# AllenInstitute/distributed-vae

Measured on AMD Instinct MI355X. Metric: cells/sec per train step (fwd+loss+bwd+opt), higher is better.
Workload: dtype f32; 1 GPU; cpl_mixVAE A=2 arms, synthetic-10x-v1 50000 cells x 5000 genes per GPU, batch 5000/GPU, fp32, H=100 L=10 C=92 S=2, x_drop=0.5, Adam lr=1e-3; global_batch=5000, parallelism=dp1, noise=in-kernel Philox4x32-10

## Files before the change

distributed-vae_amd/csrc/gemm_bf16.hip:

```cpp
#include "common.hpp"

namespace mmvae {

typedef __bf16 bf16x8 __attribute__((ext_vector_type(8)));
typedef __bf16 bf16x2 __attribute__((ext_vector_type(2)));
typedef unsigned int u32x4v __attribute__((ext_vector_type(4)));


constexpr int BT = 128;
constexpr int KT = 64;
constexpr int LDB = 36;
constexpr int LDK = 136;

template <int NP>
struct Eng {
    static constexpr int KT = NP == 1 ? 64 : 32;
    static constexpr int NQ = KT / 8;
    static constexpr int LDB = KT / 2 + 4;
    static constexpr int PLANE = BT * LDB;
    static constexpr int LDK = NP == 1 ? 136 : 160;
    static constexpr int NBUF = NP == 1 ? 2 : 1;
};

__device__ __forceinline__ unsigned pack_bf16(float a, float b) {
    bf16x2 v;
    v[0] = (__bf16)a;
    v[1] = (__bf16)b;
    return __builtin_bit_cast(unsigned, v);
}

struct Operand {
    const float* ptr;
    int64_t ld;
    int rows, K;
    int kminor;
    const uint32_t* bits;
    int wpr;
    int ones_row;
    const unsigned short* pl;
    int64_t pl_plane, pl_arm;
    int pl_ld;
    const unsigned* rowmap;
    int64_t nrec;
    int map_n;
    int src16;
};

template <bool BITS, int NQ = 8>
struct TileRegsT {
    float4 v[NQ];
    uint32_t wd[BITS ? NQ : 1];
};

struct OperandDev {
    __amdgpu_buffer_rsrc_t rs, rb;
    __amdgpu_buffer_rsrc_t rm;
    const unsigned* mp;
    int ld, rows, K, wpr, ones_row;
    bool bits;
    float4 bn_sub, bn_mul;
};
template <bool KMINOR>
__device__ __forceinline__ OperandDev make_operand_dev(const Operand& o) {
    OperandDev d;
    const int64_t n = KMINOR ? (int64_t)o.K * o.ld : (int64_t)o.rows * o.ld;
    d.rs = __builtin_amdgcn_make_buffer_rsrc(const_cast<float*>(o.ptr), 0, (int)((o.rowmap ? o.nrec : n) * (o.src16 ? 2 : 4)), 0x00020000);
    d.rm = __builtin_amdgcn_make_buffer_rsrc(const_cast<unsigned*>(o.rowmap ? o.rowmap : reinterpret_cast<const unsigned*>(o.ptr)), 0,
                                             (int)((o.rowmap ? o.map_n : 1) * 4), 0x00020000);
    d.mp = o.rowmap;
    d.bits = o.bits != nullptr;
    const int64_t nb = (KMINOR ? (int64_t)o.K : (int64_t)o.rows) * o.wpr;
    d.rb = __builtin_amdgcn_make_buffer_rsrc(const_cast<uint32_t*>(d.bits ? o.bits : reinterpret_cast<const uint32_t*>(o.ptr)), 0,
                                             (int)((d.bits ? nb : 1) * 4), 0x00020000);
    d.ld = (int)o.ld; d.rows = o.rows; d.K = o.K; d.wpr = o.wpr; d.ones_row = o.ones_row;
    return d;
}

template <bool KMINOR, int NP>
__device__ __forceinline__ void piece_ph(int q, int& p, int& h) {
    if (!KMINOR && NP != 1) { p = q; h = 0; }
    else { p = q >> 1; h = q & 1; }
}
template <bool KMINOR, bool BITS = true, int NP = 1>
__device__ __forceinline__ void quad_load(TileRegsT<BITS, Eng<NP>::NQ>& t, const OperandDev& o, int r0, int k0, int kend, int q) {
    const int tid = threadIdx.x & 255;
    int p, h;
    piece_ph<KMINOR, NP>(q, p, h);
    int off, woff;
    if (!KMINOR) {
        const int row = r0 + (tid >> 3) + 32 * p;
        const int rc = min(row, o.rows - 1);
        const int k = k0 + ((tid & 7) + 8 * h) * 4;
        const bool ok = row < o.rows && k + 3 < kend && k + 3 < o.K;
        off = rc * o.ld + (ok ? k : 0);
        woff = rc * o.wpr + ((ok ? k : 0) >> 5);
    } else {
        const int k = k0 + 2 * ((tid >> 5) + 8 * p) + h;
        const int kc = min(k, o.K - 1);
        const int row = r0 + (tid & 31) * 4;
        off = kc * o.ld + (row < o.ld ? row : 0);
        woff = kc * o.wpr + (min(row, o.rows - 1) >> 5);
    }
    t.v[q] = __builtin_bit_cast(float4, __builtin_amdgcn_raw_buffer_load_b128(o.rs, off * 4, 0, 0));
    if constexpr (BITS) t.wd[q] = o.bits ? (uint32_t)__builtin_amdgcn_raw_buffer_load_b32(o.rb, woff * 4, 0, 0) : 0xFFFFFFFFu;
}

template <bool KMINOR, int NP>
__device__ __forceinline__ void quad_load_idx(TileRegsT<true, Eng<NP>::NQ>& t, const OperandDev& o, int r0, int k0, int kend, int q,
                                              const unsigned (&ro)[Eng<NP>::NQ]) {
    const int tid = threadIdx.x & 255;
    int p, h;
    piece_ph<KMINOR, NP>(q, p, h);
    int off, woff;
    if (!KMINOR) {
        const int row = r0 + (tid >> 3) + 32 * p;
        const int rc = min(row, o.rows - 1);
        const int k = k0 + ((tid & 7) + 8 * h) * 4;
        const bool ok = row < o.rows && k + 3 < kend && k + 3 < o.K;
        off = (int)ro[q] + (ok ? k : 0);
        woff = rc * o.wpr + ((ok ? k : 0) >> 5);
    } else {
        const int k = k0 + 2 * ((tid >> 5) + 8 * p) + h;
        const int kc = min(k, o.K - 1);
        const int row = r0 + (tid & 31) * 4;
        off = (int)ro[q] + (row < o.ld ? row : 0);
        woff = kc * o.wpr + (min(row, o.rows - 1) >> 5);
    }
    t.v[q] = __builtin_bit_cast(float4, __builtin_amdgcn_raw_buffer_load_b128(o.rs, off * 4, 0, 0));
    t.wd[q] = o.bits ? (uint32_t)__builtin_amdgcn_raw_buffer_load_b32(o.rb, woff * 4, 0, 0) : 0xFFFFFFFFu;
}
typedef unsigned mapw4 __attribute__((ext_vector_type(4)));
typedef const mapw4 __attribute__((address_space(4)))* map4_ptr;
template <int NP>
struct MapRegs { mapw4 s[Eng<NP>::KT / 16]; };
template <int NP>
__device__ __forceinline__ void map_request(MapRegs<NP>& mr, const OperandDev& o, int k0) {
    const int wv = __builtin_amdgcn_readfirstlane((int)(threadIdx.x & 255) >> 6);
    const unsigned* base = o.mp + __builtin_amdgcn_readfirstlane(k0) + 4 * wv;
#pragma unroll
    for (int p = 0; p < Eng<NP>::KT / 16; ++p) mr.s[p] = *(map4_ptr)(const void*)(base + 16 * p);
}
template <int NP>
__device__ __forceinline__ void map_offsets(unsigned (&ro)[Eng<NP>::NQ], const MapRegs<NP>& mr) {
    const bool hi = (threadIdx.x & 32) != 0;
#pragma unroll
    for (int q = 0; q < Eng<NP>::NQ; ++q) {
        const int p = q >> 1, h = q & 1;
        ro[q] = hi ? mr.s[p][2 + h] : mr.s[p][h];
    }
}
template <int NP>
__device__ __forceinline__ void ro_init(unsigned (&ro)[Eng<NP>::NQ], const OperandDev& o, int r0) {
    const int tid = threadIdx.x & 255;
#pragma unroll
    for (int q = 0; q < Eng<NP>::NQ; ++q) {
        int p, h;
        piece_ph<false, NP>(q, p, h);
        ro[q] = (unsigned)__builtin_amdgcn_raw_buffer_load_b32(o.rm, min(r0 + (tid >> 3) + 32 * p, o.rows - 1) * 4, 0, 0);
    }
}
template <bool KMINOR, int NP>
__device__ __forceinline__ void idx_begin(unsigned (&ro)[Eng<NP>::NQ], MapRegs<NP>& mr, const OperandDev& o, int r0, int kfirst) {
    if constexpr (KMINOR) {
        map_request<NP>(mr, o, kfirst);
        map_offsets<NP>(ro, mr);
        map_request<NP>(mr, o, kfirst + Eng<NP>::KT);
    } else ro_init<NP>(ro, o, r0);
}
template <bool KMINOR, int NP>
__device__ __forceinline__ void idx_next(unsigned (&ro)[Eng<NP>::NQ], MapRegs<NP>& mr, const OperandDev& o, int kld) {
    if constexpr (KMINOR) {
        map_offsets<NP>(ro, mr);
        map_request<NP>(mr, o, kld + Eng<NP>::KT);
    }
}
template <bool KMINOR, bool BITS = true, int NP = 1, bool BN = false>
__device__ __forceinline__ void quad_store(unsigned* __restrict__ T, const TileRegsT<BITS, Eng<NP>::NQ>& t, const OperandDev& o, int r0,
                                           int k0, int kend, int q) {
    constexpr int LDBv = Eng<NP>::LDB, PLANE = Eng<NP>::PLANE;
    const int tid = threadIdx.x & 255;
    int p, h;
    piece_ph<KMINOR, NP>(q, p, h);
    float x[4];
    int idx;
    if (!KMINOR) {
        const int kq = tid & 7, rr = tid >> 3;
        const int row = r0 + rr + 32 * p;
        const int k = k0 + (kq + 8 * h) * 4;
        const bool ok = row < o.rows && k + 3 < kend && k + 3 < o.K;
        const int nib = ok ? (BITS ? (int)(t.wd[q] >> (k & 31)) : 0xF) : 0;
        const float4 v = t.v[q];
        const float vv[4] = {v.x, v.y, v.z, v.w};
#pragma unroll
        for (int e = 0; e < 4; ++e) x[e] = __uint_as_float(__float_as_uint(vv[e]) & (unsigned)__builtin_amdgcn_sbfe(nib, e, 1));
        idx = (rr + 32 * p) * LDBv + (kq + 8 * h) * 2;
    } else {
        const int r4 = (tid & 31) * 4, kp = tid >> 5;
        const int kl = 2 * (kp + 8 * p) + h, k = k0 + kl;
        const bool kok = k < kend && k < o.K;
        const int nrow = min(max(o.rows - (r0 + r4), 0), 4);
        const int nib = kok ? ((BITS ? (int)(t.wd[q] >> ((r0 + r4) & 31)) : 0xF) & ((1 << nrow) - 1)) : 0;
        const float4 v = t.v[q];
        const float vv[4] = {v.x, v.y, v.z, v.w};
#pragma unroll
        for (int e = 0; e < 4; ++e) x[e] = __uint_as_float(__float_as_uint(vv[e]) & (unsigned)__builtin_amdgcn_sbfe(nib, e, 1));
        if constexpr (BN) {
            const float sb[4] = {o.bn_sub.x, o.bn_sub.y, o.bn_sub.z, o.bn_sub.w}, ml[4] = {o.bn_mul.x, o.bn_mul.y, o.bn_mul.z, o.bn_mul.w};
#pragma unroll
            for (int e = 0; e < 4; ++e) x[e] = ((nib >> e) & 1) ? (x[e] - sb[e]) * ml[e] : 0.f;
        }
        if (o.ones_row >= 0) {
#pragma unroll
            for (int e = 0; e < 4; ++e)
                if (kok && r0 + r4 + e == o.ones_row) x[e] = 1.f;
        }
        idx = (kl * Eng<NP>::LDK + r4) >> 1;
    }
    if constexpr (NP == 1) {
        uint2 w;
        w.x = pack_bf16(x[0], x[1]);
        w.y = pack_bf16(x[2], x[3]);
        *reinterpret_cast<uint2*>(&T[idx]) = w;
    } else {
        unsigned w0[3], w1[3];
        split3(x[0], x[1], w0);
        split3(x[2], x[3], w1);
#pragma unroll
        for (int pl = 0; pl < 3; ++pl) *reinterpret_cast<uint2*>(&T[pl * PLANE + idx]) = make_uint2(w0[pl], w1[pl]);
    }
}

struct OctRegs { u32x4v v[4]; uint32_t wd[4]; };
template <bool KMINOR, bool IDX>
__device__ __forceinline__ void oct_load(OctRegs& t, const OperandDev& o, int r0, int k0, int kend, int p, const unsigned (&ro)[8]) {
    const int tid = threadIdx.x & 255;
    int off, woff;
    if (!KMINOR) {
        const int row = r0 + (tid >> 3) + 32 * p;
        const int rc = min(row, o.rows - 1);
        const int k = k0 + 8 * (tid & 7);
        const bool ok = row < o.rows && k + 7 < kend && k + 7 < o.K;
        off = (IDX ? (int)ro[p] : rc * o.ld) + (ok ? k : 0);
        woff = rc * o.wpr + ((ok ? k : 0) >> 5);
    } else {
        const int k = k0 + (tid >> 4) + 16 * p;
        const int kc = min(k, o.K - 1);
        const int row = r0 + 8 * (tid & 15);
        off = (IDX ? (int)ro[p] : kc * o.ld) + (row < o.ld ? row : 0);
        woff = kc * o.wpr + (min(row, o.rows - 1) >> 5);
    }
    t.v[p] = __builtin_bit_cast(u32x4v, __builtin_amdgcn_raw_buffer_load_b128(o.rs, off * 2, 0, 0));
    t.wd[p] = o.bits ? (uint32_t)__builtin_amdgcn_raw_buffer_load_b32(o.rb, woff * 4, 0, 0) : 0xFFFFFFFFu;
}
template <bool KMINOR>
__device__ __forceinline__ void oct_store(unsigned* __restrict__ T, const OctRegs& t, const OperandDev& o, int r0, int k0, int kend, int p) {
    const int tid = threadIdx.x & 255;
    int byte, idx;
    if (!KMINOR) {
        const int rr = (tid >> 3) + 32 * p, row = r0 + rr;
        const int k = k0 + 8 * (tid & 7);
        const bool ok = row < o.rows && k + 7 < kend && k + 7 < o.K;
        byte = ok ? (int)((t.wd[p] >> (k & 31)) & 0xFFu) : 0;
        idx = rr * LDB + 4 * (tid & 7);
    } else {
        const int kl = (tid >> 4) + 16 * p, k = k0 + kl;
        const int r8 = 8 * (tid & 15);
        const bool kok = k < kend && k < o.K;
        const int nrow = min(max(o.rows - (r0 + r8), 0), 8);
        byte = kok ? (int)((t.wd[p] >> ((r0 + r8) & 31)) & ((1u << nrow) - 1u)) : 0;
        idx = (kl * LDK + r8) >> 1;
    }
    u32x4v w;
#pragma unroll
    for (int j = 0; j < 4; ++j) {
        const unsigned m = ((unsigned)__builtin_amdgcn_sbfe(byte, 2 * j, 1) & 0xFFFFu) | ((unsigned)__builtin_amdgcn_sbfe(byte, 2 * j + 1, 1) & 0xFFFF0000u);
        w[j] = t.v[p][j] & m;
    }
    *reinterpret_cast<u32x4v*>(&T[idx]) = w;
}
__device__ __forceinline__ void oct_ro_init(unsigned (&ro)[8], const OperandDev& o, int r0) {
    const int tid = threadIdx.x & 255;
#pragma unroll
    for (int p = 0; p < 4; ++p) ro[p] = (unsigned)__builtin_amdgcn_raw_buffer_load_b32(o.rm, min(r0 + (tid >> 3) + 32 * p, o.rows - 1) * 4, 0, 0);
}
__device__ __forceinline__ void oct_map_offsets(unsigned (&ro)[8], const MapRegs<1>& mr) {
    const int qq = (threadIdx.x >> 4) & 3;
#pragma unroll
    for (int p = 0; p < 4; ++p) {
        const unsigned lo = (qq & 1) ? mr.s[p][1] : mr.s[p][0], hi = (qq & 1) ? mr.s[p][3] : mr.s[p][2];
        ro[p] = (qq & 2) ? hi : lo;
    }
}

template <bool KMINOR, bool BITS = true, int NP = 1>
__device__ __forceinline__ void tile_load(TileRegsT<BITS, Eng<NP>::NQ>& t, const OperandDev& o, int r0, int k0, int kend) {
#pragma unroll
    for (int q = 0; q < Eng<NP>::NQ; ++q) quad_load<KMINOR, BITS, NP>(t, o, r0, k0, kend, q);
}
template <bool KMINOR, bool BITS = true, int NP = 1>
__device__ __forceinline__ void tile_store(unsigned* __restrict__ T, const TileRegsT<BITS, Eng<NP>::NQ>& t, const OperandDev& o, int r0,
                                           int k0, int kend) {
#pragma unroll
    for (int q = 0; q < Eng<NP>::NQ; ++q) quad_store<KMINOR, BITS, NP>(T, t, o, r0, k0, kend, q);
}

typedef short s16x4 __attribute__((ext_vector_type(4)));
template <bool MINOR, int LDBv = LDB, int LDKv = LDK>
__device__ __forceinline__ bf16x8 frag8(const unsigned* T, int rb, int s, int lane) {
    if (!MINOR) {
        return __builtin_bit_cast(bf16x8, *reinterpret_cast<const u32x4v*>(T + (rb + (lane & 31)) * LDBv + 4 * (lane >> 5) + 8 * s));
    } else {
        const unsigned short* Tk = reinterpret_cast<const unsigned short*>(T);
        const int grp = lane >> 4, q = (lane & 15) >> 2, p = lane & 3;
        const unsigned short* a = Tk + (16 * s + 8 * (grp >> 1) + q) * LDKv + rb + 16 * (grp & 1) + 4 * p;
        typedef s16x4 __attribute__((address_space(3))) * lds_ptr;
        const s16x4 v0 = __builtin_amdgcn_ds_read_tr16_b64_v4i16((lds_ptr)a);
        const s16x4 v1 = __builtin_amdgcn_ds_read_tr16_b64_v4i16((lds_ptr)(a + 4 * LDKv));
        typedef short s16x8 __attribute__((ext_vector_type(8)));
        s16x8 r;
        r[0] = v0[0]; r[1] = v0[1]; r[2] = v0[2]; r[3] = v0[3];
        r[4] = v1[0]; r[5] = v1[1]; r[6] = v1[2]; r[7] = v1[3];
        return __builtin_bit_cast(bf16x8, r);
    }
}

struct PlaneRegs { u32x4v v[6]; };
struct PlaneDev { __amdgpu_buffer_rsrc_t rs; int plane, ld; };
__device__ __forceinline__ PlaneDev make_plane_dev(const Operand& o, int arm) {
    PlaneDev d;
    d.rs = __builtin_amdgcn_make_buffer_rsrc(const_cast<unsigned short*>(o.pl + (int64_t)arm * o.pl_arm), 0, (int)(3 * o.pl_plane * 2), 0x00020000);
    d.plane = (int)o.pl_plane; d.ld = o.pl_ld;
    return d;
}
template <bool KMINOR>
__device__ __forceinline__ void plane_load(PlaneRegs& t, const PlaneDev& o, int r0, int k0, int j) {
    const int tid = threadIdx.x & 255, pl = j >> 1, id = tid + 256 * (j & 1);
    int off;
    if (!KMINOR) off = pl * o.plane + (r0 + (id >> 2)) * o.ld + k0 + 8 * (id & 3);
    else off = pl * o.plane + (k0 + (id >> 4)) * o.ld + r0 + 8 * (id & 15);
    t.v[j] = __builtin_bit_cast(u32x4v, __builtin_amdgcn_raw_buffer_load_b128(o.rs, off * 2, 0, 0));
}
template <bool KMINOR>
__device__ __forceinline__ void plane_store(unsigned* __restrict__ T, const PlaneRegs& t, int j) {
    const int tid = threadIdx.x & 255, pl = j >> 1, id = tid + 256 * (j & 1);
    int idx;
    if (!KMINOR) idx = pl * Eng<3>::PLANE + (id >> 2) * Eng<3>::LDB + 4 * (id & 3);
    else idx = pl * Eng<3>::PLANE + (((id >> 4) * Eng<3>::LDK + 8 * (id & 15)) >> 1);
    *reinterpret_cast<u32x4v*>(&T[idx]) = t.v[j];
}

struct SplitJob {
    const float* src; int64_t ld, src_arm;
    int R, C, Rp, Cp, ones_col;
    unsigned short* dst; int64_t dst_arm;
    const float* col_src; int64_t col_arm;
    int tr;
};
struct XbitsJob {
    NoiseDev nz; int A, B, D, wpr; uint32_t* bits; int blocks; float* zero_p; int zero_n4;
    const int64_t* rows; unsigned* map; int64_t rows_ld, n_rows;
};
struct SplitJobs { SplitJob j[24]; int first[25]; int n; XbitsJob xb; };
__global__ __launch_bounds__(256) void k_presplit(const SplitJobs js) {
    if (js.xb.zero_n4 > 0) grid_zero(js.xb.zero_p, js.xb.zero_n4);
    if (js.xb.rows && blockIdx.z == 0) {
        for (int i = blockIdx.x * 256 + threadIdx.x; i < js.xb.B + MAP_PAD; i += gridDim.x * 256) {
            const int64_t r = i < js.xb.B ? js.xb.rows[i] : 0;
            js.xb.map[i] = (unsigned)((r < 0 ? 0 : (r >= js.xb.n_rows ? js.xb.n_rows - 1 : r)) * js.xb.rows_ld);
        }
    }
    if ((int)blockIdx.x < js.xb.blocks) {
        make_xbits_range(js.xb.nz, js.xb.A, js.xb.B, js.xb.D, js.xb.wpr, js.xb.bits,
                         ((int64_t)blockIdx.z * js.xb.blocks + blockIdx.x) * 256 + threadIdx.x, (int64_t)gridDim.z * js.xb.blocks * 256);
        return;
    }
    const int bx0 = (int)blockIdx.x - js.xb.blocks;
    int ji = 0;
    while (ji + 1 < js.n && bx0 >= js.first[ji + 1]) ++ji;
    const SplitJob& J = js.j[ji];
    const int bx = bx0 - js.first[ji], nbx = js.first[ji + 1] - js.first[ji];
    const float* src = J.src + (int64_t)blockIdx.z * J.src_arm;
    const float* col = J.col_src ? J.col_src + (int64_t)blockIdx.z * J.col_arm : nullptr;
    unsigned short* dst = J.dst + (int64_t)blockIdx.z * J.dst_arm;
    const int c8n = J.Cp >> 3;
    const int64_t plane = (int64_t)J.Rp * J.Cp;
    const bool vec = (J.ld & 3) == 0 && (J.C & 3) == 0;
    const int n = J.Rp * c8n;
    for (int i = bx * 256 + threadIdx.x; i < n; i += nbx * 256) {
        const int r = i / c8n, c0 = (i - r * c8n) * 8;
        float v[8];
        if (J.tr) {
#pragma unroll
            for (int e = 0; e < 8; ++e) v[e] = (r < J.R && c0 + e < J.C) ? src[(int64_t)(c0 + e) * J.ld + r] : 0.f;
        } else if (r < J.R && vec && c0 + 8 <= J.C) {
            const float4 a = *reinterpret_cast<const float4*>(src + (int64_t)r * J.ld + c0);
            const float4 b = *reinterpret_cast<const float4*>(src + (int64_t)r * J.ld + c0 + 4);
            v[0] = a.x; v[1] = a.y; v[2] = a.z; v[3] = a.w; v[4] = b.x; v[5] = b.y; v[6] = b.z; v[7] = b.w;
        } else {
#pragma unroll
            for (int e = 0; e < 8; ++e) {
                const int c = c0 + e;
                v[e] = (r < J.R && c < J.C) ? src[(int64_t)r * J.ld + c] : ((r < J.R && c == J.ones_col) ? (col ? col[r] : 1.f) : 0.f);
            }
        }
        unsigned w[4][3];
#pragma unroll
        for (int e = 0; e < 4; ++e) split3(v[2 * e], v[2 * e + 1], w[e]);
#pragma unroll
        for (int pl = 0; pl < 3; ++pl)
            *reinterpret_cast<uint4*>(dst + pl * plane + (int64_t)r * J.Cp + c0) = make_uint4(w[0][pl], w[1][pl], w[2][pl], w[3][pl]);
    }
}

struct SlabOut {
    float* out;
    int64_t ks_stride, arm_stride;
    int ld, M, N;
};
struct Fc11Out {
    const float* bias;
    const float* x;
    float* dz;
    float* x_rec;
    float* part;
    float coef;
    int B, D;
    const unsigned* xmap;
    int64_t x_nrec;
};

struct GemmArgs {
    Operand a, b;
    int64_t a_arm, b_arm;
    int64_t a_bits_arm, b_bits_arm;
    int64_t bias_arm;
    int M, N, K;
    int KS;
    SlabOut so;
    Fc11Out fo;
    int64_t fo_arm, fo_x_arm;
    int n11;
    int A;
};

template <bool AMINOR, bool BMINOR, int NP = 1>
__device__ __forceinline__ void mfma_ktile(f32x16 (&acc)[2][2], const unsigned* As, const unsigned* Bs, int wm, int wn, int lane) {
    constexpr int LDBv = Eng<NP>::LDB, PLANE = Eng<NP>::PLANE, NS = Eng<NP>::KT / 16;
    bf16x8 a[NP == 3 ? 2 : 1][2][NP], b[NP == 3 ? 2 : 1][2][NP];
    auto frags = [&](int s, int w) __attribute__((always_inline)) {
#pragma unroll
        for (int pl = 0; pl < NP; ++pl) {
            a[w][0][pl] = frag8<AMINOR, LDBv, Eng<NP>::LDK>(As + pl * PLANE, wm * 64, s, lane);
            a[w][1][pl] = frag8<AMINOR, LDBv, Eng<NP>::LDK>(As + pl * PLANE, wm * 64 + 32, s, lane);
            b[w][0][pl] = frag8<BMINOR, LDBv, Eng<NP>::LDK>(Bs + pl * PLANE, wn * 64, s, lane);
            b[w][1][pl] = frag8<BMINOR, LDBv, Eng<NP>::LDK>(Bs + pl * PLANE, wn * 64 + 32, s, lane);
        }
    };
    if constexpr (NP == 3) {
        frags(0, 0);
        frags(1, 1);
        __builtin_amdgcn_sched_barrier(0);
    }
#pragma unroll
    for (int s = 0; s < NS; ++s) {
        const int w = NP == 3 ? s : 0;
        if constexpr (NP != 3) frags(s, 0);
#pragma unroll
        for (int i = 0; i < 2; ++i)
#pragma unroll
            for (int j = 0; j < 2; ++j) {
                if constexpr (NP == 3) {
                    acc[i][j] = __builtin_amdgcn_mfma_f32_32x32x16_bf16(a[w][i][2], b[w][j][0], acc[i][j], 0, 0, 0);
                    acc[i][j] = __builtin_amdgcn_mfma_f32_32x32x16_bf16(a[w][i][0], b[w][j][2], acc[i][j], 0, 0, 0);
                    acc[i][j] = __builtin_amdgcn_mfma_f32_32x32x16_bf16(a[w][i][1], b[w][j][1], acc[i][j], 0, 0, 0);
                    acc[i][j] = __builtin_amdgcn_mfma_f32_32x32x16_bf16(a[w][i][1], b[w][j][0], acc[i][j], 0, 0, 0);
                    acc[i][j] = __builtin_amdgcn_mfma_f32_32x32x16_bf16(a[w][i][0], b[w][j][1], acc[i][j], 0, 0, 0);
                }
                acc[i][j] = __builtin_amdgcn_mfma_f32_32x32x16_bf16(a[w][i][0], b[w][j][0], acc[i][j], 0, 0, 0);
            }
    }
}

__device__ __forceinline__ void gemm_epilogue(const GemmArgs& g, const f32x16 (&acc)[2][2], int m0, int n0, int wm, int wn, int lane, int arm) {
    const int l31 = lane & 31;
    float* out = g.so.out + (int64_t)blockIdx.y * g.so.ks_stride + (int64_t)arm * g.so.arm_stride;
#pragma unroll
    for (int i = 0; i < 2; ++i)
#pragma unroll
        for (int j = 0; j < 2; ++j) {
            const int col = n0 + 64 * wn + 32 * j + l31;
#pragma unroll
            for (int r = 0; r < 16; ++r) {
                const int row = m0 + 64 * wm + 32 * i + acc_row(r, lane);
                if (row < g.so.M && col < g.so.N) out[(int64_t)row * g.so.ld + col] = acc[i][j][r];
            }
        }
}

template <bool AMINOR, bool BMINOR, int IDX = 0, int S16 = 0>
__global__ __launch_bounds__(256, 2) void k_bf16_gemm(const GemmArgs g_in) {
    const GemmArgs g = g_in;
    __shared__ __attribute__((aligned(16))) unsigned As[2][BT * LDB];
    __shared__ __attribute__((aligned(16))) unsigned Bs[2][BT * LDB];
    const int arm = blockIdx.z, tid = threadIdx.x, lane = tid & 63, wv = tid >> 6, wm = wv >> 1, wn = wv & 1;
    Operand oa_h = g.a, ob_h = g.b;
    oa_h.ptr += (int64_t)arm * g.a_arm;
    ob_h.ptr += (int64_t)arm * g.b_arm;
    if (oa_h.bits) oa_h.bits += (int64_t)arm * g.a_bits_arm;
    if (ob_h.bits) ob_h.bits += (int64_t)arm * g.b_bits_arm;
    const OperandDev oa = make_operand_dev<AMINOR>(oa_h), ob = make_operand_dev<BMINOR>(ob_h);
    const int tiles_n = cdiv(g.N, BT);
    const int wg = blockIdx.x;
    const int m0 = (wg / tiles_n) * BT, n0 = (wg % tiles_n) * BT;
    const int nkt = cdiv(g.K, KT);
    const int kb = (int)(((int64_t)blockIdx.y * nkt) / g.KS) * KT;
    const int ke = min(g.K, (int)(((int64_t)(blockIdx.y + 1) * nkt) / g.KS) * KT);
    f32x16 acc[2][2] = {{zero16(), zero16()}, {zero16(), zero16()}};
    TileRegsT<true> ta, tb;
    OctRegs t16a, t16b;
    unsigned ro[Eng<1>::NQ] = {};
    MapRegs<1> mr = {};
    static_assert(IDX == 0 || S16 == 0 || (S16 & IDX) != 0, "row map and bf16 storage: the indexed operand (x) is a bf16 one");
    constexpr bool A16 = (S16 & 1) != 0, B16 = (S16 & 2) != 0;
    auto stage = [&](unsigned* Ad, unsigned* Bd, int kst, int kld, auto load_tag) __attribute__((always_inline)) {
        constexpr bool LOAD = decltype(load_tag)::value;
        if constexpr (LOAD && IDX == 1 && AMINOR) {
            if constexpr (A16) { oct_map_offsets(ro, mr); map_request<1>(mr, oa, kld + KT); }
            else idx_next<AMINOR, 1>(ro, mr, oa, kld);
        }
        if constexpr (LOAD && IDX == 2 && BMINOR) {
            if constexpr (B16) { oct_map_offsets(ro, mr); map_request<1>(mr, ob, kld + KT); }
            else idx_next<BMINOR, 1>(ro, mr, ob, kld);
        }
#pragma unroll
        for (int q = 0; q < 8; ++q) {
            if constexpr (A16) {
                if (q < 4) {
                    oct_store<AMINOR>(Ad, t16a, oa, m0, kst, ke, q);
                    if constexpr (LOAD) oct_load<AMINOR, IDX == 1>(t16a, oa, m0, kld, ke, q, ro);
                }
            } else {
                quad_store<AMINOR>(Ad, ta, oa, m0, kst, ke, q);
                if constexpr (LOAD) {
                    if constexpr (IDX == 1) quad_load_idx<AMINOR, 1>(ta, oa, m0, kld, ke, q, ro);
                    else quad_load<AMINOR>(ta, oa, m0, kld, ke, q);
                }
            }
            if constexpr (B16) {
                if (q < 4) {
                    oct_store<BMINOR>(Bd, t16b, ob, n0, kst, ke, q);
                    if constexpr (LOAD) oct_load<BMINOR, IDX == 2>(t16b, ob, n0, kld, ke, q, ro);
                }
            } else {
                quad_store<BMINOR>(Bd, tb, ob, n0, kst, ke, q);
                if constexpr (LOAD) {
                    if constexpr (IDX == 2) quad_load_idx<BMINOR, 1>(tb, ob, n0, kld, ke, q, ro);
                    else quad_load<BMINOR>(tb, ob, n0, kld, ke, q);
                }
            }
        }
    };
    auto first = [&](auto a_tag) __attribute__((always_inline)) {
        constexpr bool ISA = decltype(a_tag)::value;
        constexpr bool MINOR = ISA ? AMINOR : BMINOR;
        constexpr bool IDXD = IDX == (ISA ? 1 : 2), IS16 = ISA ? A16 : B16;
        const OperandDev& o = ISA ? oa : ob;
        const int r0 = ISA ? m0 : n0;
        OctRegs& t16 = ISA ? t16a : t16b;
        if constexpr (IS16) {
            if constexpr (IDXD) {
                if constexpr (MINOR) { map_request<1>(mr, o, kb); oct_map_offsets(ro, mr); map_request<1>(mr, o, kb + KT); }
                else oct_ro_init(ro, o, r0);
            }
#pragma unroll
            for (int q = 0; q < 4; ++q) oct_load<MINOR, IDXD>(t16, o, r0, kb, ke, q, ro);
        } else if constexpr (IDXD) {
            idx_begin<MINOR, 1>(ro, mr, o, r0, kb);
#pragma unroll
            for (int q = 0; q < Eng<1>::NQ; ++q) quad_load_idx<MINOR, 1>(ISA ? ta : tb, o, r0, kb, ke, q, ro);
        } else tile_load<MINOR>(ISA ? ta : tb, o, r0, kb, ke);
    };
    if (kb < ke) {
        first(VecTag{});
        first(ScalarTag{});
    }
    if (kb < ke) {
        if (kb + KT < ke) stage(As[0], Bs[0], kb, kb + KT, VecTag{});
        else stage(As[0], Bs[0], kb, kb, ScalarTag{});
    }
    __syncthreads();
    int cur = 0;
    for (int k0 = kb; k0 < ke; k0 += KT) {
        mfma_ktile<AMINOR, BMINOR>(acc, As[cur], Bs[cur], wm, wn, lane);
        if (k0 + 2 * KT < ke) stage(As[cur ^ 1], Bs[cur ^ 1], k0 + KT, k0 + 2 * KT, VecTag{});
        else if (k0 + KT < ke) stage(As[cur ^ 1], Bs[cur ^ 1], k0 + KT, k0 + KT, ScalarTag{});
        __syncthreads();
        cur ^= 1;
    }
    gemm_epilogue(g, acc, m0, n0, wm, wn, lane, arm);
}

#ifndef X3_DEPTH
#define X3_DEPTH 1
#endif
static_assert(X3_DEPTH == 1 || X3_DEPTH == 2, "one or two K tiles in flight");
template <bool AMINOR, bool BMINOR, int SHARE, int IDX = 0>
__global__ __launch_bounds__(512, 1) void k_x3_gemm(const GemmArgs g_in) {
    static_assert(SHARE == 1 || SHARE == 2, "the two tiles of a block share one operand");
    typedef Eng<3> E;
    constexpr int KTv = E::KT;
    const GemmArgs g = g_in;
    __shared__ __attribute__((aligned(16))) unsigned As[2][3 * E::PLANE];
    __shared__ __attribute__((aligned(16))) unsigned Bs[2][3 * E::PLANE];
    const int arm = blockIdx.z, grp = threadIdx.x >> 8, tid = threadIdx.x & 255, lane = tid & 63, wv = tid >> 6, wm = wv >> 1, wn = wv & 1;
    Operand oa_h = g.a, ob_h = g.b;
    oa_h.ptr += (int64_t)arm * g.a_arm;
    ob_h.ptr += (int64_t)arm * g.b_arm;
    if (oa_h.bits) oa_h.bits += (int64_t)arm * g.a_bits_arm;
    if (ob_h.bits) ob_h.bits += (int64_t)arm * g.b_bits_arm;
    const OperandDev oa = make_operand_dev<AMINOR>(oa_h), ob = make_operand_dev<BMINOR>(ob_h);
    const int tiles_m = cdiv(g.M, BT), tiles_n = cdiv(g.N, BT);
    const int bi = blockIdx.x;
    int tm, tn;
    if (SHARE == 2) { tn = bi % tiles_n; tm = 2 * (bi / tiles_n) + grp; }
    else { tm = bi % tiles_m; tn = 2 * (bi / tiles_m) + grp; }
    const bool active = tm < tiles_m && tn < tiles_n;
    const int m0 = tm * BT, n0 = tn * BT;
    const int nkt = cdiv(g.K, KTv);
    const int kb = (int)(((int64_t)blockIdx.y * nkt) / g.KS) * KTv;
    const int ke = min(g.K, (int)(((int64_t)(blockIdx.y + 1) * nkt) / g.KS) * KTv);
    const int n = ke > kb ? cdiv(ke - kb, KTv) : 0;
    f32x16 acc[2][2] = {{zero16(), zero16()}, {zero16(), zero16()}};
    constexpr int DEPTH = X3_DEPTH;
    TileRegsT<true, E::NQ> ta_[DEPTH], tb_[DEPTH];
    unsigned ro[E::NQ] = {};
    MapRegs<3> mr = {};
    PlaneRegs ps;
    constexpr bool APL = SHARE == 1, BPL = SHARE == 2;
    const PlaneDev dp = make_plane_dev(SHARE == 1 ? g.a : g.b, arm);
    const bool do_a = SHARE != 1 || grp == 0, do_b = SHARE != 2 || grp == 0;
    auto stage = [&](unsigned* Ad, unsigned* Bd, int kst, int kld, int kpl, auto load_tag, auto loadp_tag, auto slot_tag) __attribute__((always_inline)) {
        constexpr bool LOAD = decltype(load_tag)::value, LOADP = decltype(loadp_tag)::value;
        constexpr int SLOT = decltype(slot_tag)::value;
        TileRegsT<true, E::NQ>& ta = ta_[SLOT];
        TileRegsT<true, E::NQ>& tb = tb_[SLOT];
        if constexpr (LOAD && IDX == 1) idx_next<AMINOR, 3>(ro, mr, oa, kld);
        if constexpr (LOAD && IDX == 2) idx_next<BMINOR, 3>(ro, mr, ob, kld);
#pragma unroll
        for (int i = 0; i < 6; ++i) {
            if constexpr (APL) {
                if (do_a) {
                    plane_store<AMINOR>(Ad, ps, i);
                    if constexpr (LOADP) plane_load<AMINOR>(ps, dp, m0, kpl, i);
                }
            } else if (i < E::NQ) {
                if (do_a) {
                    quad_store<AMINOR, true, 3>(Ad, ta, oa, m0, kst, ke, i);
                    if constexpr (LOAD) {
                        if constexpr (IDX == 1) quad_load_idx<AMINOR, 3>(ta, oa, m0, kld, ke, i, ro);
                        else quad_load<AMINOR, true, 3>(ta, oa, m0, kld, ke, i);
                    }
                }
            }
            if constexpr (BPL) {
                if (do_b) {
                    plane_store<BMINOR>(Bd, ps, i);
                    if constexpr (LOADP) plane_load<BMINOR>(ps, dp, n0, kpl, i);
                }
            } else if (i < E::NQ) {
                if (do_b) {
                    quad_store<BMINOR, true, 3>(Bd, tb, ob, n0, kst, ke, i);
                    if constexpr (LOAD) {
                        if constexpr (IDX == 2) quad_load_idx<BMINOR, 3>(tb, ob, n0, kld, ke, i, ro);
                        else quad_load<BMINOR, true, 3>(tb, ob, n0, kld, ke, i);
                    }
                }
            }
        }
    };
    auto first = [&](auto slot_tag, int k) __attribute__((always_inline)) {
        constexpr int SLOT = decltype(slot_tag)::value;
        TileRegsT<true, E::NQ>& ta = ta_[SLOT];
        TileRegsT<true, E::NQ>& tb = tb_[SLOT];
        if constexpr (APL) {
            if (SLOT == 0 && do_a) {
#pragma unroll
                for (int i = 0; i < 6; ++i) plane_load<AMINOR>(ps, dp, m0, k, i);
            }
        } else if (do_a) {
            if constexpr (IDX == 1) {
                if constexpr (SLOT == 0) idx_begin<AMINOR, 3>(ro, mr, oa, m0, k);
                else idx_next<AMINOR, 3>(ro, mr, oa, k);
#pragma unroll
                for (int q = 0; q < E::NQ; ++q) quad_load_idx<AMINOR, 3>(ta, oa, m0, k, ke, q, ro);
            } else tile_load<AMINOR, true, 3>(ta, oa, m0, k, ke);
        }
        if constexpr (BPL) {
            if (SLOT == 0 && do_b) {
#pragma unroll
                for (int i = 0; i < 6; ++i) plane_load<BMINOR>(ps, dp, n0, k, i);
            }
        } else if (do_b) {
            if constexpr (IDX == 2) {
                if constexpr (SLOT == 0) idx_begin<BMINOR, 3>(ro, mr, ob, n0, k);
                else idx_next<BMINOR, 3>(ro, mr, ob, k);
#pragma unroll
                for (int q = 0; q < E::NQ; ++q) quad_load_idx<BMINOR, 3>(tb, ob, n0, k, ke, q, ro);
            } else tile_load<BMINOR, true, 3>(tb, ob, n0, k, ke);
        }
    };
    if (active && n > 0) {
        first(std::integral_constant<int, 0>{}, kb);
        if constexpr (DEPTH > 1) {
            if (n > 1) first(std::integral_constant<int, DEPTH - 1>{}, kb + KTv);
        }
    }
    for (int p = 0; p <= 2 * n; ++p) {
        const int q = p - grp;
        if (active && q >= 0 && q < 2 * n) {
            const int t = q >> 1, k0 = kb + t * KTv;
            unsigned* const Ad = As[SHARE == 1 ? (t & 1) : grp];
            unsigned* const Bd = Bs[SHARE == 2 ? (t & 1) : grp];
            if (q & 1) {
                mfma_ktile<AMINOR, BMINOR, 3>(acc, Ad, Bd, wm, wn, lane);
            } else {
                const bool more = t + DEPTH < n, morep = t + 1 < n;
                const int kld = k0 + DEPTH * KTv, kpl = k0 + KTv;
                auto go = [&](auto slot_tag) __attribute__((always_inline)) {
                    if (more) stage(Ad, Bd, k0, kld, kpl, VecTag{}, VecTag{}, slot_tag);
                    else if (morep) stage(Ad, Bd, k0, k0, kpl, ScalarTag{}, VecTag{}, slot_tag);
                    else stage(Ad, Bd, k0, k0, k0, ScalarTag{}, ScalarTag{}, slot_tag);
                };
                if (DEPTH == 1 || !(t & 1)) go(std::integral_constant<int, 0>{});
                else go(std::integral_constant<int, DEPTH - 1>{});
            }
        }
        __syncthreads();
    }
    if (active) gemm_epilogue(g, acc, m0, n0, wm, wn, lane, arm);
}

__global__ __launch_bounds__(256, 2) void k_bf16_fc11(const GemmArgs g_in) {
    const GemmArgs g = g_in;
    __shared__ __attribute__((aligned(16))) unsigned Ws[2][BT * LDB];
    __shared__ __attribute__((aligned(16))) unsigned Ds[2][BT * LDB];
    __shared__ float red[8];
    const int arm = blockIdx.z, tid = threadIdx.x, lane = tid & 63, wv = tid >> 6, wm = wv >> 1, wn = wv & 1;
    const int l31 = lane & 31, hh = lane >> 5;
    Operand od_h = g.a, ow_h = g.b;
    od_h.ptr += (int64_t)arm * g.a_arm;
    ow_h.ptr += (int64_t)arm * g.b_arm;
    const OperandDev od = make_operand_dev<false>(od_h), ow = make_operand_dev<false>(ow_h);
    const int c0 = blockIdx.x * BT;
    const int tiles = cdiv(g.N, BT);
    const int t0 = (int)(((int64_t)blockIdx.y * tiles) / g.KS), t1 = (int)(((int64_t)(blockIdx.y + 1) * tiles) / g.KS);
    const int K = g.K;
    const float* xa = g.fo.x + (int64_t)arm * g.fo_x_arm;
    float* dza = g.fo.dz + (int64_t)arm * g.fo_arm;
    float* xra = g.fo.x_rec ? g.fo.x_rec + (int64_t)arm * g.fo_arm : nullptr;
    const float* bias = g.fo.bias + (int64_t)arm * g.bias_arm;
    const int B = g.fo.B, D = g.fo.D;
    {
        TileRegsT<false> t0r, t1r;
        tile_load<false, false>(t0r, od, c0, 0, K);
        tile_load<false, false>(t1r, od, c0, KT, K);
        tile_store<false, false>(Ds[0], t0r, od, c0, 0, K);
        tile_store<false, false>(Ds[1], t1r, od, c0, KT, K);
    }
    TileRegsT<false> w0, w1;
    if (t0 < t1) {
        tile_load<false, false>(w0, ow, t0 * BT, 0, K);
        tile_load<false, false>(w1, ow, t0 * BT, KT, K);
    }
    float se = 0.f;
    int mism = 0;
    for (int t = t0; t < t1; ++t) {
        const int j0 = t * BT;
        tile_store<false, false>(Ws[0], w0, ow, j0, 0, K);
        tile_store<false, false>(Ws[1], w1, ow, j0, KT, K);
        __syncthreads();
        if (t + 1 < t1) {
            tile_load<false, false>(w0, ow, j0 + BT, 0, K);
            tile_load<false, false>(w1, ow, j0 + BT, KT, K);
        }
        float4 xin[2][4], b4[2][4];
        auto request = [&](int pc, float4 (&X)[4], float4 (&Bq)[4]) __attribute__((always_inline)) {
            const int i = pc >> 1, j = pc & 1;
            const int cell = c0 + 64 * wn + 32 * j + l31;
            const int64_t rowoff = (int64_t)min(cell, B - 1) * D;
#pragma unroll
            for (int q = 0; q < 4; ++q) {
                const int gene = j0 + 64 * wm + 32 * i + 8 * q + 4 * hh;
                const int gc = min(gene, D - 4);
                X[q] = *reinterpret_cast<const float4*>(xa + rowoff + gc);
                Bq[q] = *reinterpret_cast<const float4*>(bias + gc);
            }
        };
        request(0, xin[0], b4[0]);
        __builtin_amdgcn_sched_barrier(0);
        f32x16 acc[2][2] = {{zero16(), zero16()}, {zero16(), zero16()}};
        mfma_ktile<false, false>(acc, Ws[0], Ds[0], wm, wn, lane);
        if (K > KT) mfma_ktile<false, false>(acc, Ws[1], Ds[1], wm, wn, lane);
#pragma unroll
        for (int pc = 0; pc < 4; ++pc) {
            const int i = pc >> 1, j = pc & 1;
            if (pc + 1 < 4) request(pc + 1, xin[(pc + 1) & 1], b4[(pc + 1) & 1]);
            __builtin_amdgcn_sched_barrier(0);
            const int cell = c0 + 64 * wn + 32 * j + l31;
#pragma unroll
            for (int q = 0; q < 4; ++q) {
                const int gene = j0 + 64 * wm + 32 * i + 8 * q + 4 * hh;
                const bool ok = cell < B && gene < D;
                const float4 xq = xin[pc & 1][q], bq = b4[pc & 1][q];
                const float xv[4] = {xq.x, xq.y, xq.z, xq.w};
                const float bv[4] = {bq.x, bq.y, bq.z, bq.w};
                float xr[4], dz[4];
#pragma unroll
                for (int e = 0; e < 4; ++e) {
                    xr[e] = fmaxf(acc[i][j][4 * q + e] + bv[e], 0.f);
                    const float er = xr[e] - xv[e];
                    dz[e] = xr[e] > 0.f ? g.fo.coef * er : 0.f;
                    se += ok ? er * er : 0.f;
                    mism += (ok && ((xr[e] > 0.1f) != (xv[e] > 0.1f))) ? 1 : 0;
                }
                if (ok) {
                    *reinterpret_cast<float4*>(dza + (int64_t)cell * D + gene) = make_float4(dz[0], dz[1], dz[2], dz[3]);
                    if (xra) *reinterpret_cast<float4*>(xra + (int64_t)cell * D + gene) = make_float4(xr[0], xr[1], xr[2], xr[3]);
                }
            }
            asm volatile("" : "+v"(mism), "+v"(se));
            __builtin_amdgcn_sched_barrier(0);
        }
        __syncthreads();
    }
    se = wave_sum(se);
    const float mf = wave_sum((float)mism);
    if (lane == 0) { red[wv * 2] = se; red[wv * 2 + 1] = mf; }
    __syncthreads();
    if (tid == 0) {
        float* p = g.fo.part + ((int64_t)arm * g.n11 + (int64_t)blockIdx.x * g.KS + blockIdx.y) * 2;
        p[0] = red[0] + red[2] + red[4] + red[6];
        p[1] = red[1] + red[3] + red[5] + red[7];
    }
}

static_assert(KT == 64, "W16: a row of W11's planes (128 bf16) is exactly the two K tiles in LDS");
template <bool S16, bool W16 = false>
__global__ __launch_bounds__(256, 2) void k_bf16_fc11g(const GemmArgs g_in) {
    const GemmArgs g = g_in;
    __shared__ __attribute__((aligned(16))) unsigned Ws[2][BT * LDB];
    __shared__ __attribute__((aligned(16))) unsigned Ds[2][BT * LDB];
    __shared__ __attribute__((aligned(16))) float bias_s[BT];
    __shared__ float red[8];
    const int arm = blockIdx.z, tid = threadIdx.x, lane = tid & 63, wv = tid >> 6;
    const int l31 = lane & 31, hh = lane >> 5;
    Operand od_h = g.a, ow_h = g.b;
    od_h.ptr += (int64_t)arm * g.a_arm;
    ow_h.ptr += (int64_t)arm * g.b_arm;
    const OperandDev od = make_operand_dev<false>(od_h), ow = make_operand_dev<false>(ow_h);
    const int c0 = blockIdx.x * BT;
    const int tiles = cdiv(g.N, BT);
    const int t0 = (int)(((int64_t)blockIdx.y * tiles) / g.KS), t1 = (int)(((int64_t)(blockIdx.y + 1) * tiles) / g.KS);
    const int K = g.K;
    const int ksteps1 = K > KT ? cdiv(K - KT, 16) : 0;
    const float* xa = g.fo.x + (int64_t)arm * g.fo_x_arm;
    float* dza = g.fo.dz + (int64_t)arm * g.fo_arm;
    const float* bias = g.fo.bias + (int64_t)arm * g.bias_arm;
    const int B = g.fo.B, D = g.fo.D;
    {
        TileRegsT<false> t0r, t1r;
        tile_load<false, false>(t0r, od, c0, 0, K);
        tile_load<false, false>(t1r, od, c0, KT, K);
        tile_store<false, false>(Ds[0], t0r, od, c0, 0, K);
        tile_store<false, false>(Ds[1], t1r, od, c0, KT, K);
    }
    TileRegsT<false> w0, w1;
    OctRegs wo0, wo1;
    const unsigned no_map[8] = {0, 0, 0, 0, 0, 0, 0, 0};
    auto w_request = [&](int j) __attribute__((always_inline)) {
        if constexpr (W16) {
#pragma unroll
            for (int p = 0; p < 4; ++p) {
                oct_load<false, false>(wo0, ow, j, 0, 2 * KT, p, no_map);
                oct_load<false, false>(wo1, ow, j, KT, 2 * KT, p, no_map);
            }
        } else {
            tile_load<false, false>(w0, ow, j, 0, K);
            tile_load<false, false>(w1, ow, j, KT, K);
        }
    };
    auto w_store = [&](int j) __attribute__((always_inline)) {
        if constexpr (W16) {
#pragma unroll
            for (int p = 0; p < 4; ++p) {
                oct_store<false>(Ws[0], wo0, ow, j, 0, 2 * KT, p);
                oct_store<false>(Ws[1], wo1, ow, j, KT, 2 * KT, p);
            }
        } else {
            tile_store<false, false>(Ws[0], w0, ow, j, 0, K);
            tile_store<false, false>(Ws[1], w1, ow, j, KT, K);
        }
    };
    float bnext = 0.f;
    if (t0 < t1) {
        w_request(t0 * BT);
        if (tid < BT) bnext = bias[min(t0 * BT + tid, D - 1)];
    }
    f32x16 gd[4] = {zero16(), zero16(), zero16(), zero16()};
    float se = 0.f;
    int mism = 0;
    const int cell = c0 + 32 * wv + l31;
    const int64_t rowoff = g.fo.xmap ? (int64_t)g.fo.xmap[min(cell, B - 1)] : (int64_t)min(cell, B - 1) * D;
    const unsigned short* Wk16[2] = {reinterpret_cast<const unsigned short*>(Ws[0]), reinterpret_cast<const unsigned short*>(Ws[1])};
    typedef short s16x4 __attribute__((ext_vector_type(4)));
    typedef s16x4 __attribute__((address_space(3))) * lds_ptr;
    const int tr_off = ((lane & 15) >> 2) * (2 * LDB) + 16 * ((lane >> 4) & 1) + 4 * (lane & 3);
    for (int t = t0; t < t1; ++t) {
        const int j0 = t * BT;
        w_store(j0);
        if (tid < BT) bias_s[tid] = bnext;
        __syncthreads();
        if (t + 1 < t1) {
            w_request(j0 + BT);
            if (tid < BT) bnext = bias[min(j0 + BT + tid, D - 1)];
        }
#pragma unroll
        for (int half = 0; half < 2; ++half) {
            float4 xin[2][4];
            u32x4v xraw[2][2];
#pragma unroll
            for (int gl = 0; gl < 2; ++gl) {
                if constexpr (S16) {
#pragma unroll
                    for (int qp = 0; qp < 2; ++qp) {
                        const int gene = j0 + 32 * (2 * half + gl) + 8 * (2 * qp + hh);
                        xraw[gl][qp] = *reinterpret_cast<const u32x4v*>(reinterpret_cast<const unsigned short*>(xa) + rowoff + min(gene, D - 8));
                    }
                } else {
#pragma unroll
                    for (int q = 0; q < 4; ++q) {
                        const int gene = j0 + 32 * (2 * half + gl) + 8 * q + 4 * hh;
                        xin[gl][q] = *reinterpret_cast<const float4*>(xa + rowoff + min(gene, D - 4));
                    }
                }
            }
            __builtin_amdgcn_sched_barrier(0);
            f32x16 acc[2] = {zero16(), zero16()};
#pragma unroll
            for (int s = 0; s < KT / 16; ++s) {
                const bf16x8 b = frag8<false>(Ds[0], 32 * wv, s, lane);
                acc[0] = __builtin_amdgcn_mfma_f32_32x32x16_bf16(frag8<false>(Ws[0], 32 * (2 * half), s, lane), b, acc[0], 0, 0, 0);
                acc[1] = __builtin_amdgcn_mfma_f32_32x32x16_bf16(frag8<false>(Ws[0], 32 * (2 * half + 1), s, lane), b, acc[1], 0, 0, 0);
            }
            for (int s = 0; s < ksteps1; ++s) {
                const bf16x8 b = frag8<false>(Ds[1], 32 * wv, s, lane);
                acc[0] = __builtin_amdgcn_mfma_f32_32x32x16_bf16(frag8<false>(Ws[1], 32 * (2 * half), s, lane), b, acc[0], 0, 0, 0);
                acc[1] = __builtin_amdgcn_mfma_f32_32x32x16_bf16(frag8<false>(Ws[1], 32 * (2 * half + 1), s, lane), b, acc[1], 0, 0, 0);
            }
#pragma unroll
            for (int gl = 0; gl < 2; ++gl) {
                const int gi = 2 * half + gl;
                float dzr[16];
                if constexpr (S16) {
#pragma unroll
                    for (int qp = 0; qp < 2; ++qp) {
                        const auto s0 = __builtin_amdgcn_permlane32_swap(xraw[gl][qp][0], xraw[gl][qp][2], false, false);
                        const auto s1 = __builtin_amdgcn_permlane32_swap(xraw[gl][qp][1], xraw[gl][qp][3], false, false);
                        xin[gl][2 * qp] = make_float4(__uint_as_float(s0[0] << 16), __uint_as_float(s0[0] & 0xFFFF0000u),
                                                      __uint_as_float(s1[0] << 16), __uint_as_float(s1[0] & 0xFFFF0000u));
                        xin[gl][2 * qp + 1] = make_float4(__uint_as_float(s0[1] << 16), __uint_as_float(s0[1] & 0xFFFF0000u),
                                                          __uint_as_float(s1[1] << 16), __uint_as_float(s1[1] & 0xFFFF0000u));
                    }
                }
#pragma unroll
                for (int q = 0; q < 4; ++q) {
                    const int gene = j0 + 32 * gi + 8 * q + 4 * hh;
                    const bool ok = cell < B && gene < D;
                    const float4 xq = xin[gl][q];
                    const float4 bq = *reinterpret_cast<const float4*>(&bias_s[32 * gi + 8 * q + 4 * hh]);
                    const float xv[4] = {xq.x, xq.y, xq.z, xq.w};
                    const float bv[4] = {bq.x, bq.y, bq.z, bq.w};
#pragma unroll
                    for (int e = 0; e < 4; ++e) {
                        const float xr = fmaxf(acc[gl][4 * q + e] + bv[e], 0.f);
                        const float er = xr - xv[e];
                        dzr[4 * q + e] = (ok && xr > 0.f) ? g.fo.coef * er : 0.f;
                        se += ok ? er * er : 0.f;
                        mism += (ok && ((xr > 0.1f) != (xv[e] > 0.1f))) ? 1 : 0;
                    }
                    if constexpr (!S16) {
                        if (ok) *reinterpret_cast<float4*>(dza + (int64_t)cell * D + gene) =
                            make_float4(dzr[4 * q], dzr[4 * q + 1], dzr[4 * q + 2], dzr[4 * q + 3]);
                    }
                }
                if constexpr (S16) {
#pragma unroll
                    for (int qp = 0; qp < 2; ++qp) {
                        const int qe = 2 * qp, qo = 2 * qp + 1;
                        const auto s0 = __builtin_amdgcn_permlane32_swap(pack_bf16(dzr[4 * qe], dzr[4 * qe + 1]), pack_bf16(dzr[4 * qo], dzr[4 * qo + 1]), false, false);
                        const auto s1 = __builtin_amdgcn_permlane32_swap(pack_bf16(dzr[4 * qe + 2], dzr[4 * qe + 3]), pack_bf16(dzr[4 * qo + 2], dzr[4 * qo + 3]), false, false);
                        u32x4v w;
                        w[0] = s0[0]; w[1] = s1[0]; w[2] = s0[1]; w[3] = s1[1];
                        const int gene = j0 + 32 * gi + 8 * (2 * qp + hh);
                        if (cell < B && gene < D) *reinterpret_cast<u32x4v*>(reinterpret_cast<unsigned short*>(dza) + (int64_t)cell * D + gene) = w;
                    }
                }
#pragma unroll
                for (int c = 0; c < 2; ++c) {
                    u32x4v au;
                    au[0] = pack_bf16(dzr[8 * c + 0], dzr[8 * c + 1]);
                    au[1] = pack_bf16(dzr[8 * c + 2], dzr[8 * c + 3]);
                    au[2] = pack_bf16(dzr[8 * c + 4], dzr[8 * c + 5]);
                    au[3] = pack_bf16(dzr[8 * c + 6], dzr[8 * c + 7]);
                    const bf16x8 afr = __builtin_bit_cast(bf16x8, au);
                    const int grow = 32 * gi + 16 * c + 4 * hh;
#pragma unroll
                    for (int nt = 0; nt < 4; ++nt) {
                        const unsigned short* a = Wk16[nt >> 1] + grow * (2 * LDB) + 32 * (nt & 1) + tr_off;
                        const s16x4 v0 = __builtin_amdgcn_ds_read_tr16_b64_v4i16((lds_ptr)a);
                        const s16x4 v1 = __builtin_amdgcn_ds_read_tr16_b64_v4i16((lds_ptr)(a + 8 * (2 * LDB)));
                        typedef short s16x8 __attribute__((ext_vector_type(8)));
                        s16x8 r;
                        r[0] = v0[0]; r[1] = v0[1]; r[2] = v0[2]; r[3] = v0[3];
                        r[4] = v1[0]; r[5] = v1[1]; r[6] = v1[2]; r[7] = v1[3];
                        gd[nt] = __builtin_amdgcn_mfma_f32_32x32x16_bf16(afr, __builtin_bit_cast(bf16x8, r), gd[nt], 0, 0, 0);
                    }
                }
                asm volatile("" : "+v"(mism), "+v"(se));
                __builtin_amdgcn_sched_barrier(0);
            }
        }
        __syncthreads();
    }
    {
        const int H = g.K;
        float* out = g.so.out + (int64_t)blockIdx.y * g.so.ks_stride + (int64_t)arm * g.so.arm_stride;
#pragma unroll
        for (int nt = 0; nt < 4; ++nt) {
            const int h = 32 * nt + l31;
#pragma unroll
            for (int r = 0; r < 16; ++r) {
                const int row = c0 + 32 * wv + acc_row(r, lane);
                if (row < B && h < H) out[(int64_t)row * H + h] = gd[nt][r];
            }
        }
    }
    se = wave_sum(se);
    const float mf = wave_sum((float)mism);
    if (lane == 0) { red[wv * 2] = se; red[wv * 2 + 1] = mf; }
    __syncthreads();
    if (tid == 0) {
        float* p = g.fo.part + ((int64_t)arm * g.n11 + (int64_t)blockIdx.x * g.KS + blockIdx.y) * 2;
        p[0] = red[0] + red[2] + red[4] + red[6];
        p[1] = red[1] + red[3] + red[5] + red[7];
    }
}

constexpr int FW_ROW = 64;
constexpr int FW_PLANE = 64 * FW_ROW;
constexpr int FW_TILE = 3 * FW_PLANE;
__device__ __forceinline__ int fw_swz(int row) { return ((row & 3) << 2) | ((row >> 2) & 3); }
__global__ __launch_bounds__(256, 1) void k_x3_fc11g(const GemmArgs g_in) {
    const GemmArgs g = g_in;
    __shared__ __attribute__((aligned(16))) unsigned Wl[3 * FW_TILE];
    __shared__ float red[8];
    const int arm = blockIdx.z, tid = threadIdx.x, lane = tid & 63, wv = tid >> 6;
    const int l31 = lane & 31, hh = lane >> 5;
    const unsigned short* Wp = g.b.pl + (int64_t)arm * g.b.pl_arm;
    const unsigned short* Dp = g.a.pl + (int64_t)arm * g.a.pl_arm;
    const int64_t wplane = g.b.pl_plane, dplane = g.a.pl_plane;
    const int B = g.fo.B, D = g.fo.D, H = g.K;
    const int c0 = blockIdx.x * 128;
    const int tiles = cdiv(D, 64);
    const int t0 = (int)(((int64_t)blockIdx.y * tiles) / g.KS), t1 = (int)(((int64_t)(blockIdx.y + 1) * tiles) / g.KS);
    const int cell = c0 + 32 * wv + l31;
    const float* xa = g.fo.x + (int64_t)arm * g.fo_x_arm;
    float* dza = g.fo.dz + (int64_t)arm * g.fo_arm;
    const __amdgpu_buffer_rsrc_t rx = __builtin_amdgcn_make_buffer_rsrc(const_cast<float*>(xa), 0, (int)((g.fo.xmap ? g.fo.x_nrec : (int64_t)B * D) * 4), 0x00020000);
    const __amdgpu_buffer_rsrc_t rz = __builtin_amdgcn_make_buffer_rsrc(dza, 0, (int)((int64_t)B * D * 4), 0x00020000);
    const int rowoff = g.fo.xmap ? (int)g.fo.xmap[min(cell, B - 1)] : min(cell, B - 1) * D;
    const bool cell_ok = cell < B;
    int dzoff = min(cell, B - 1) * D * 4;
    asm volatile("" : "+v"(dzoff));
    int dlim = cell_ok ? D : 0;
    asm volatile("" : "+v"(dlim));

    const int wv_s = __builtin_amdgcn_readfirstlane(wv);
    const unsigned wl_base = (unsigned)(size_t)(__attribute__((address_space(3))) void*)(&Wl[0]);
    const int lrow = 4 * wv + (lane >> 4);
    const unsigned dma_voff = 2u * ((unsigned)lrow * 128u + 8u * (unsigned)((lane & 15) ^ fw_swz(lrow)));
    auto dma = [&](int t) __attribute__((always_inline)) {
        const int buf = (t - t0) % 3;
        const unsigned lds0 = wl_base + 4u * (unsigned)(buf * FW_TILE) + 1024u * (unsigned)wv_s;
        const unsigned short* src0 = Wp + (int64_t)t * (64 * 128);
#pragma unroll
        for (int j = 0; j < 12; ++j) {
            const unsigned short* src = src0 + (int64_t)(j >> 2) * wplane + (j & 3) * (16 * 128);
            const unsigned lds_addr = lds0 + 4u * (unsigned)((j >> 2) * FW_PLANE) + 4096u * (unsigned)(j & 3);
            asm volatile("s_mov_b32 m0, %0\n\ts_nop 0\n\tglobal_load_lds_dwordx4 %1, %2"
                         :: "s"(lds_addr), "v"(dma_voff), "s"(src) : "memory");
        }
    };
    if (t0 < t1) dma(t0);
    if (t0 + 1 < t1) dma(t0 + 1);
    bf16x8 dfr[7][3];
    {
        const int cr = min(cell, (int)(dplane / 128) - 1);
#pragma unroll
        for (int s = 0; s < 7; ++s)
#pragma unroll
            for (int pl = 0; pl < 3; ++pl)
                dfr[s][pl] = __builtin_bit_cast(bf16x8, *reinterpret_cast<const u32x4v*>(Dp + (int64_t)pl * dplane + (int64_t)cr * 128 + 16 * s + 8 * hh));
    }
    f32x16 gd[4] = {zero16(), zero16(), zero16(), zero16()};
    float seq[4] = {0.f, 0.f, 0.f, 0.f};
    int mism = 0;
    typedef s16x4 __attribute__((address_space(3))) * lds_ptr;
    typedef short s16x8 __attribute__((ext_vector_type(8)));
    const int tr_q = (lane & 15) >> 2, tr_blk = 2 * ((lane >> 4) & 1) + ((lane & 3) >> 1), tr_half = 4 * (lane & 1);
    const int npieces = 2 * (t1 - t0);
    auto w_rows = [&](int p) __attribute__((always_inline)) { return Wl + ((p >> 1) % 3) * FW_TILE + 32 * (p & 1) * FW_ROW; };
    const int a_swz = fw_swz(l31);
    auto a_frag = [&](const unsigned* Wr, int s, int pl) __attribute__((always_inline)) {
        return __builtin_bit_cast(bf16x8, *reinterpret_cast<const u32x4v*>(Wr + pl * FW_PLANE + l31 * FW_ROW + 4 * ((2 * s + hh) ^ a_swz)));
    };
    auto request_x = [&](float4 (&X)[4], int j0g, int q) __attribute__((always_inline)) {
        const int gene = j0g + 8 * q + 4 * hh;
        int off = gene < dlim ? (rowoff + gene) * 4 : -16;
        asm("" : "+v"(off));
        X[q] = __builtin_bit_cast(float4, __builtin_amdgcn_raw_buffer_load_b128(rx, off, 0, 0));
    };
    auto mfma6 = [&](f32x16& acc, const bf16x8 (&a)[3], int s) __attribute__((always_inline)) {
        acc = __builtin_amdgcn_mfma_f32_32x32x16_bf16(a[2], dfr[s][0], acc, 0, 0, 0);
        acc = __builtin_amdgcn_mfma_f32_32x32x16_bf16(a[0], dfr[s][2], acc, 0, 0, 0);
        acc = __builtin_amdgcn_mfma_f32_32x32x16_bf16(a[1], dfr[s][1], acc, 0, 0, 0);
        acc = __builtin_amdgcn_mfma_f32_32x32x16_bf16(a[1], dfr[s][0], acc, 0, 0, 0);
        acc = __builtin_amdgcn_mfma_f32_32x32x16_bf16(a[0], dfr[s][1], acc, 0, 0, 0);
        acc = __builtin_amdgcn_mfma_f32_32x32x16_bf16(a[0], dfr[s][0], acc, 0, 0, 0);
    };
    bf16x8 an[3][3];
    bf16x8 wq[2][2][3];
    auto z_frags = [&](const unsigned* Wr, int s) __attribute__((always_inline)) {
#pragma unroll
        for (int pl = 0; pl < 3; ++pl) an[s % 3][pl] = a_frag(Wr, s, pl);
    };
    auto d_frags = [&](const unsigned short* Wt16, int r) __attribute__((always_inline)) {
        const int row0 = 16 * (r >> 1) + 4 * hh + tr_q;
        const int sw0 = fw_swz(row0), sw1 = fw_swz(row0 + 8);
#pragma unroll
        for (int j = 0; j < 2; ++j)
#pragma unroll
            for (int pl = 0; pl < 3; ++pl) {
                const int blk = 4 * (2 * (r & 1) + j) + tr_blk;
                const unsigned short* base = Wt16 + pl * (2 * FW_PLANE) + tr_half;
                const s16x4 v0 = __builtin_amdgcn_ds_read_tr16_b64_v4i16((lds_ptr)(base + row0 * (2 * FW_ROW) + 8 * (blk ^ sw0)));
                const s16x4 v1 = __builtin_amdgcn_ds_read_tr16_b64_v4i16((lds_ptr)(base + (row0 + 8) * (2 * FW_ROW) + 8 * (blk ^ sw1)));
                s16x8 rr;
                rr[0] = v0[0]; rr[1] = v0[1]; rr[2] = v0[2]; rr[3] = v0[3];
                rr[4] = v1[0]; rr[5] = v1[1]; rr[6] = v1[2]; rr[7] = v1[3];
                wq[r & 1][j][pl] = __builtin_bit_cast(bf16x8, rr);
            }
    };
    float4 xa_[4], xb_[4];
    f32x16 acc_a = zero16();
    __builtin_amdgcn_s_waitcnt(0x0F70);
#pragma unroll
    for (int s7 = 0; s7 < 7; ++s7)
#pragma unroll
        for (int pl = 0; pl < 3; ++pl) asm volatile("" : "+a"(dfr[s7][pl]));
    if (npieces > 0) {
#pragma unroll
        for (int q = 0; q < 4; ++q) request_x(xa_, t0 * 64, q);
        __builtin_amdgcn_s_waitcnt(0x0F70);
#pragma unroll
        for (int q = 0; q < 4; ++q) asm volatile("" : "+v"(xa_[q].x), "+v"(xa_[q].y), "+v"(xa_[q].z), "+v"(xa_[q].w));
        __syncthreads();
        if (t0 + 2 < t1) dma(t0 + 2);
        const unsigned* Wr = w_rows(0);
#pragma unroll
        for (int s = 0; s < 7; ++s) {
            bf16x8 a[3];
#pragma unroll
            for (int pl = 0; pl < 3; ++pl) a[pl] = a_frag(Wr, s, pl);
            mfma6(acc_a, a, s);
        }
        const unsigned* W1 = w_rows(npieces > 1 ? 1 : 0);
        z_frags(W1, 0);
        z_frags(W1, 1);
    }
    auto piece = [&](int p, f32x16& accn, float4 (&xin)[4], float4 (&xnx)[4], int dma_tile) __attribute__((always_inline)) {
        const int j0g = t0 * 64 + 32 * p;
        const unsigned* Wn = w_rows(p + 1 < npieces ? p + 1 : p);
        const unsigned short* Wt16 = reinterpret_cast<const unsigned short*>(w_rows(p));
        f32x16 acc = accn;
        asm volatile("" : "+v"(acc));
        accn = zero16();
        unsigned au[2][3][4];
        float dzq[4];
#pragma unroll
        for (int q = 0; q < 4; ++q) request_x(xnx, j0g + 32, q);
        auto chunk = [&](int ch) __attribute__((always_inline)) {
            const int q = ch >> 1;
            if ((ch & 1) == 0) {
                const int gene = j0g + 8 * q + 4 * hh;
                const float xv[4] = {xin[q].x, xin[q].y, xin[q].z, xin[q].w};
#pragma unroll
                for (int e = 0; e < 4; ++e) {
                    const float a_ = acc[4 * q + e];
                    const float xr = __int_as_float(max(__float_as_int(a_), 0));
                    const float er = xr - xv[e];
                    seq[q] = __builtin_fmaf(er, er, seq[q]);
                    const float d_ = g.fo.coef * er;
                    dzq[e] = a_ > 0.f ? d_ : 0.f;
                    mism += __builtin_popcountll(__builtin_amdgcn_ballot_w64(xr > 0.1f) ^ __builtin_amdgcn_ballot_w64(xv[e] > 0.1f));
                }
                int soff = gene < dlim ? dzoff + gene * 4 : -16;
                asm("" : "+v"(soff));
                __builtin_amdgcn_raw_buffer_store_b128(__builtin_bit_cast(u32x4v, make_float4(dzq[0], dzq[1], dzq[2], dzq[3])), rz, soff, 0, 0);
            } else {
                unsigned w0[3], w1[3];
                split3(dzq[0], dzq[1], w0);
                split3(dzq[2], dzq[3], w1);
#pragma unroll
                for (int pl = 0; pl < 3; ++pl) { au[q >> 1][pl][2 * (q & 1)] = w0[pl]; au[q >> 1][pl][2 * (q & 1) + 1] = w1[pl]; }
            }
        };
#pragma unroll
        for (int q = 0; q < 4; ++q) asm volatile("" : "+v"(xin[q].x), "+v"(xin[q].y), "+v"(xin[q].z), "+v"(xin[q].w));
#pragma unroll
        for (int s = 0; s < 7; ++s) {
            __builtin_amdgcn_sched_barrier(0);
            if (s + 2 < 7) z_frags(Wn, s + 2);
            if (s == 5) d_frags(Wt16, 0);
            mfma6(accn, an[s % 3], s);
            if (s < 5) chunk(s);
        }
        asm volatile("" : "+s"(mism));
        if (dma_tile >= 0) dma(dma_tile);
#pragma unroll
        for (int r = 0; r < 4; ++r) {
            __builtin_amdgcn_sched_barrier(0);
            if (r + 1 < 4) d_frags(Wt16, r + 1);
            if (r >= 2) {
                const unsigned* W2 = w_rows(p + 2 < npieces ? p + 2 : p);
                z_frags(W2, r - 2);
            }
            if (r == 0) { chunk(5); chunk(6); }
            if (r == 1) chunk(7);
            const int c = r >> 1;
            bf16x8 af[3];
#pragma unroll
            for (int pl = 0; pl < 3; ++pl) {
                u32x4v u;
                u[0] = au[c][pl][0]; u[1] = au[c][pl][1]; u[2] = au[c][pl][2]; u[3] = au[c][pl][3];
                af[pl] = __builtin_bit_cast(bf16x8, u);
            }
            const int n0 = 2 * (r & 1);
#pragma unroll
            for (int j = 0; j < 2; ++j) gd[n0 + j] = __builtin_amdgcn_mfma_f32_32x32x16_bf16(af[2], wq[r & 1][j][0], gd[n0 + j], 0, 0, 0);
#pragma unroll
            for (int j = 0; j < 2; ++j) gd[n0 + j] = __builtin_amdgcn_mfma_f32_32x32x16_bf16(af[0], wq[r & 1][j][2], gd[n0 + j], 0, 0, 0);
#pragma unroll
            for (int j = 0; j < 2; ++j) gd[n0 + j] = __builtin_amdgcn_mfma_f32_32x32x16_bf16(af[1], wq[r & 1][j][1], gd[n0 + j], 0, 0, 0);
#pragma unroll
            for (int j = 0; j < 2; ++j) gd[n0 + j] = __builtin_amdgcn_mfma_f32_32x32x16_bf16(af[1], wq[r & 1][j][0], gd[n0 + j], 0, 0, 0);
#pragma unroll
            for (int j = 0; j < 2; ++j) gd[n0 + j] = __builtin_amdgcn_mfma_f32_32x32x16_bf16(af[0], wq[r & 1][j][1], gd[n0 + j], 0, 0, 0);
#pragma unroll
            for (int j = 0; j < 2; ++j) gd[n0 + j] = __builtin_amdgcn_mfma_f32_32x32x16_bf16(af[0], wq[r & 1][j][0], gd[n0 + j], 0, 0, 0);
        }
        __builtin_amdgcn_sched_barrier(0);
    };
    for (int t = t0; t < t1; ++t) {
        const int p = 2 * (t - t0);
        piece(p, acc_a, xa_, xb_, (t > t0 && t + 2 < t1) ? t + 2 : -1);
        piece(p + 1, acc_a, xb_, xa_, -1);
        __builtin_amdgcn_s_waitcnt(0x0F74);
        __syncthreads();
    }
    {
        float* out = g.so.out + (int64_t)blockIdx.y * g.so.ks_stride + (int64_t)arm * g.so.arm_stride;
#pragma unroll
        for (int nt = 0; nt < 4; ++nt) {
            const int h = 32 * nt + l31;
#pragma unroll
            for (int r = 0; r < 16; ++r) {
                const int row = c0 + 32 * wv + acc_row(r, lane);
                if (row < B && h < H) out[(int64_t)row * H + h] = gd[nt][r];
            }
        }
    }
    const float se = wave_sum((seq[0] + seq[1]) + (seq[2] + seq[3]));
    if (lane == 0) { red[wv * 2] = se; red[wv * 2 + 1] = (float)mism; }
    __syncthreads();
    if (tid == 0) {
        float* pp = g.fo.part + ((int64_t)arm * g.n11 + (int64_t)blockIdx.x * g.KS + blockIdx.y) * 2;
        pp[0] = (red[0] + red[2]) + (red[4] + red[6]);
        pp[1] = (red[1] + red[3]) + (red[5] + red[7]);
    }
    if (blockIdx.x == 0 && blockIdx.y == 0)
        for (int i = (int)gridDim.x * g.KS * 2 + tid; i < 2 * g.n11; i += 256) g.fo.part[(int64_t)arm * g.n11 * 2 + i] = 0.f;
}

struct Fc11OutArgs {
    const unsigned short* wpl; int64_t w_plane, w_arm;
    const unsigned short* dpl; int64_t d_plane, d_arm;
    float* out;
    int B, D, KS;
};
template <int NP, int NK>
__global__ __launch_bounds__(256, 1) void k_fc11_out(const Fc11OutArgs g) {
    const int arm = blockIdx.z, tid = threadIdx.x, lane = tid & 63, wv = tid >> 6;
    const int l31 = lane & 31, hh = lane >> 5;
    const int B = g.B, D = g.D;
    const int cell = blockIdx.x * 128 + 32 * wv + l31;
    const unsigned short* Wp = g.wpl + (int64_t)arm * g.w_arm;
    const unsigned short* Dp = g.dpl + (int64_t)arm * g.d_arm;
    bf16x8 dfr[NK][NP];
    {
        const int cr = min(cell, (int)(g.d_plane / 128) - 1);
#pragma unroll
        for (int s = 0; s < NK; ++s)
#pragma unroll
            for (int pl = 0; pl < NP; ++pl)
                dfr[s][pl] = __builtin_bit_cast(bf16x8, *reinterpret_cast<const u32x4v*>(Dp + (int64_t)pl * g.d_plane + (int64_t)cr * 128 + 16 * s + 8 * hh));
    }
    const int npc = cdiv(D, 32);
    const int p0 = (int)(((int64_t)blockIdx.y * npc) / g.KS), p1 = (int)(((int64_t)(blockIdx.y + 1) * npc) / g.KS);
    auto load_w = [&](int p, bf16x8 (&a)[NK][NP]) __attribute__((always_inline)) {
        const unsigned short* r = Wp + (int64_t)(32 * p + l31) * 128 + 8 * hh;
#pragma unroll
        for (int s = 0; s < NK; ++s)
#pragma unroll
            for (int pl = 0; pl < NP; ++pl)
                a[s][pl] = __builtin_bit_cast(bf16x8, *reinterpret_cast<const u32x4v*>(r + (int64_t)pl * g.w_plane + 16 * s));
    };
    float* orow = g.out + ((int64_t)arm * B + min(cell, B - 1)) * D;
    const bool cell_ok = cell < B;
    bf16x8 wa[NK][NP], wb[NK][NP];
    auto piece = [&](int p, const bf16x8 (&a)[NK][NP]) __attribute__((always_inline)) {
        f32x16 acc = zero16();
#pragma unroll
        for (int s = 0; s < NK; ++s) {
            if constexpr (NP == 3) {
                acc = __builtin_amdgcn_mfma_f32_32x32x16_bf16(a[s][2], dfr[s][0], acc, 0, 0, 0);
                acc = __builtin_amdgcn_mfma_f32_32x32x16_bf16(a[s][0], dfr[s][2], acc, 0, 0, 0);
                acc = __builtin_amdgcn_mfma_f32_32x32x16_bf16(a[s][1], dfr[s][1], acc, 0, 0, 0);
                acc = __builtin_amdgcn_mfma_f32_32x32x16_bf16(a[s][1], dfr[s][0], acc, 0, 0, 0);
                acc = __builtin_amdgcn_mfma_f32_32x32x16_bf16(a[s][0], dfr[s][1], acc, 0, 0, 0);
            }
            acc = __builtin_amdgcn_mfma_f32_32x32x16_bf16(a[s][0], dfr[s][0], acc, 0, 0, 0);
        }
#pragma unroll
        for (int q = 0; q < 4; ++q) {
            const int gene = 32 * p + 8 * q + 4 * hh;
            if (cell_ok && gene < D)
                *reinterpret_cast<float4*>(orow + gene) = make_float4(relu_keep_nan(acc[4 * q]), relu_keep_nan(acc[4 * q + 1]),
                                                                      relu_keep_nan(acc[4 * q + 2]), relu_keep_nan(acc[4 * q + 3]));
        }
    };
    if (p0 < p1) load_w(p0, wa);
    for (int p = p0; p < p1; p += 2) {
        if (p + 1 < p1) load_w(p + 1, wb);
        piece(p, wa);
        if (p + 1 >= p1) break;
        if (p + 2 < p1) load_w(p + 2, wa);
        piece(p + 1, wb);
    }
}

__global__ __launch_bounds__(512, 1) void k_x3_small(const TnDescs descs, int ndesc, int A, int B, int KS) {
    typedef Eng<3> E;
    constexpr int KTv = E::KT;
    __shared__ __attribute__((aligned(16))) unsigned As[2][3 * E::PLANE];
    __shared__ __attribute__((aligned(16))) unsigned Bs[2][3 * E::PLANE];
    const int grp = threadIdx.x >> 8, tid = threadIdx.x & 255, lane = tid & 63, wv = tid >> 6, wm = wv >> 1, wn = wv & 1;
    const int unit = 2 * blockIdx.x + grp;
    const bool active = unit < ndesc * A;
    const int di = active ? unit % ndesc : 0, arm = active ? unit / ndesc : 0;
    const TnDesc& dr = descs.d[di];
    const TnDesc d = {dr.P, dr.p_arm_stride, dr.ldp, dr.Mv, dr.Q, dr.q_arm_stride, dr.ldq, dr.Nv, dr.q_ones, dr.q_xmask,
                      dr.q_mean, dr.q_rstd, dr.out, dr.out_arm_stride, dr.out_ks_stride, dr.ldo};
    Operand oa_h{d.P + (int64_t)arm * d.p_arm_stride, d.ldp, d.Mv, B, 1, nullptr, 0, -1, nullptr, 0, 0, 0};
    Operand ob_h{d.Q + (int64_t)arm * d.q_arm_stride, d.ldq, d.Nv, B, 1, nullptr, 0, d.q_ones ? d.Nv : -1, nullptr, 0, 0, 0};
    OperandDev oa = make_operand_dev<true>(oa_h), ob = make_operand_dev<true>(ob_h);
    const bool bn = d.q_mean != nullptr;
    {
        const int r4 = (tid & 31) * 4;
        float sb[4] = {0.f, 0.f, 0.f, 0.f}, ml[4] = {1.f, 1.f, 1.f, 1.f};
        if (bn) {
#pragma unroll
            for (int e = 0; e < 4; ++e)
                if (r4 + e < d.Nv) { sb[e] = d.q_mean[(int64_t)arm * d.Nv + r4 + e]; ml[e] = d.q_rstd[(int64_t)arm * d.Nv + r4 + e]; }
        }
        ob.bn_sub = make_float4(sb[0], sb[1], sb[2], sb[3]);
        ob.bn_mul = make_float4(ml[0], ml[1], ml[2], ml[3]);
    }
    const int nkt = cdiv(B, KTv);
    const int kb = (int)(((int64_t)blockIdx.y * nkt) / KS) * KTv;
    const int ke = min(B, (int)(((int64_t)(blockIdx.y + 1) * nkt) / KS) * KTv);
    const int n = ke > kb ? cdiv(ke - kb, KTv) : 0;
    f32x16 acc[2][2] = {{zero16(), zero16()}, {zero16(), zero16()}};
    TileRegsT<false, E::NQ> ta, tb;
    unsigned* const Ad = As[grp];
    unsigned* const Bd = Bs[grp];
    auto stage = [&](int kst, int kld, auto load_tag) __attribute__((always_inline)) {
        constexpr bool LOAD = decltype(load_tag)::value;
#pragma unroll
        for (int i = 0; i < E::NQ; ++i) {
            quad_store<true, false, 3>(Ad, ta, oa, 0, kst, ke, i);
            if constexpr (LOAD) quad_load<true, false, 3>(ta, oa, 0, kld, ke, i);
            quad_store<true, false, 3, true>(Bd, tb, ob, 0, kst, ke, i);
            if constexpr (LOAD) quad_load<true, false, 3>(tb, ob, 0, kld, ke, i);
        }
    };
    if (active && n > 0) {
        tile_load<true, false, 3>(ta, oa, 0, kb, ke);
        tile_load<true, false, 3>(tb, ob, 0, kb, ke);
    }
    for (int p = 0; p <= 2 * n; ++p) {
        const int q = p - grp;
        if (active && q >= 0 && q < 2 * n) {
            const int k0 = kb + (q >> 1) * KTv;
            if (q & 1) mfma_ktile<true, true, 3>(acc, Ad, Bd, wm, wn, lane);
            else if (k0 + KTv < ke) stage(k0, k0 + KTv, VecTag{});
            else stage(k0, k0, ScalarTag{});
        }
        __syncthreads();
    }
    if (!active) return;
    float* out = d.out + (int64_t)blockIdx.y * d.out_ks_stride + (int64_t)arm * d.out_arm_stride;
    const int ncols = d.Nv + d.q_ones, l31 = lane & 31;
#pragma unroll
    for (int i = 0; i < 2; ++i)
#pragma unroll
        for (int j = 0; j < 2; ++j) {
            const int col = 64 * wn + 32 * j + l31;
#pragma unroll
            for (int r = 0; r < 16; ++r) {
                const int row = 64 * wm + 32 * i + acc_row(r, lane);
                if (row < d.Mv && col < ncols) out[(int64_t)row * d.ldo + col] = acc[i][j][r];
            }
        }
}

static Operand kmajor(const float* p, int64_t ld, int rows, int K) {
    Operand o{};
    o.ptr = p; o.ld = ld; o.rows = rows; o.K = K; o.ones_row = -1;
    return o;
}
static Operand kminor(const float* p, int64_t ld, int rows, int K) { Operand o = kmajor(p, ld, rows, K); o.kminor = 1; return o; }

enum { PL_W1 = 0, PL_W11 = 1, PL_D10 = 2, PL_DZ1 = 3 };
struct PlaneGeom { int R, C, Rp, Cp, ones_col; int64_t ws_off; };
static PlaneGeom plane_geom(const Ctx& c, int kind) {
    const mmvae_dims& d = c.d;
    switch (kind) {
        case PL_W1:  return PlaneGeom{d.H, d.D, 128, rup(d.D, 32), -1, c.lay.pl_w1};
        case PL_W11: return PlaneGeom{d.D, d.H, rup(d.D, 128), 128, d.H, c.lay.pl_w11};
        case PL_D10: return PlaneGeom{d.B, d.H, rup(d.B, 256), 128, d.H, c.lay.pl_d10};
        default:     return PlaneGeom{d.B, d.H, rup(d.B, 256), 128, -1, c.lay.pl_dz1};
    }
}
static void use_planes(const Ctx& c, Operand& o, int kind) {
    const PlaneGeom g = plane_geom(c, kind);
    o.pl = reinterpret_cast<const unsigned short*>(c.ws + g.ws_off);
    o.pl_plane = (int64_t)g.Rp * g.Cp; o.pl_arm = 3 * o.pl_plane; o.pl_ld = g.Cp;
}
static int64_t read_slice0_bf16(const Ctx& c, Operand& o, int kind, bool whole = false) {
    const PlaneGeom g = plane_geom(c, kind);
    o.ptr = reinterpret_cast<const float*>(c.ws + g.ws_off); o.ld = g.Cp; o.src16 = 1;
    if (whole) { o.rows = g.Rp; o.K = g.Cp; }
    return 3 * (int64_t)g.Rp * g.Cp / 2;
}
static SplitJob plane_job(const Ctx& c, int kind, const float* src, int64_t ld, int64_t src_arm, const float* col_src = nullptr, int64_t col_arm = 0) {
    const PlaneGeom g = plane_geom(c, kind);
    return SplitJob{src, ld, src_arm, g.R, g.C, g.Rp, g.Cp, g.ones_col, reinterpret_cast<unsigned short*>(c.ws + g.ws_off),
                    3 * (int64_t)g.Rp * g.Cp, col_src, col_arm};
}
static int launch_presplit(hipStream_t s, int A, const SplitJob* jobs, int n, const XbitsJob* xb = nullptr) {
    SplitJobs js{};
    if (xb) js.xb = *xb;
    js.n = n;
    for (int i = 0; i < n; ++i) {
        js.j[i] = jobs[i];
        js.first[i + 1] = js.first[i] + (int)imin64(1024, cdiv64((int64_t)jobs[i].Rp * (jobs[i].Cp / 8), 256));
    }
    hipLaunchKernelGGL(k_presplit, dim3(js.xb.blocks + js.first[n], 1, A), dim3(256), 0, s, js);
    HIP_LAUNCH_CHECK("k_presplit");
    return 0;
}

static SplitJob small_plane_job(const Ctx& c, const float* params, int s, bool transposed) {
    const int H = c.d.H, L = c.d.L, CS = c.d.C + c.d.S;
    const int ti[PL_SMALL_LAYERS] = {2, 4, 6, 8, 16, 18, 20, 22, 24};
    const int nn[PL_SMALL_LAYERS] = {H, H, H, L, L, H, H, H, H}, kk[PL_SMALL_LAYERS] = {H, H, H, H, CS, L, H, H, H};
    unsigned short* base = reinterpret_cast<unsigned short*>(c.ws + c.lay.pl_small);
    return SplitJob{params + c.po.o[ti[s]], kk[s], c.po.per_arm, transposed ? kk[s] : nn[s], transposed ? nn[s] : kk[s], 128, 128, -1,
                    base + (int64_t)(transposed ? PL_SMALL_LAYERS + s : s) * 3 * 128 * 128, (int64_t)PL_SMALL_SLOTS * 3 * 128 * 128,
                    nullptr, 0, transposed ? 1 : 0};
}

int launch_x3_planes(const Ctx& c, const float* params, bool head, const mmvae_noise* nz) {
    const Plan& p = c.plan;
    const mmvae_dims& d = c.d;
    XbitsJob xb{};
    const bool xbits = head && p.zero == ZERO_PRESPLIT;
    if (xbits) {
        xb.nz = make_noise_dev(nz, c.h);
        xb.A = d.A; xb.B = d.B; xb.D = d.D; xb.wpr = cdiv(d.D, 32);
        xb.bits = reinterpret_cast<uint32_t*>(c.ws + c.lay.xbits);
        xb.blocks = (int)imin64(2048, cdiv64((int64_t)d.B * cdiv(xb.wpr, xbits_words_per_thread(xb.nz)), 256));
        xb.zero_p = c.ws + c.lay.fc11_part;
        xb.zero_n4 = (int)(c.fwd_zero_floats() / 4);
        if (p.rowmap) {
            xb.rows = c.x_rows; xb.map = reinterpret_cast<unsigned*>(c.ws + c.lay.rowmap);
            xb.rows_ld = c.x_ld; xb.n_rows = c.x_nrows;
        }
    }
    SplitJob jobs[24];
    int n = 0;
    if (head && (p.big == GEMM_X3 || p.narrow)) {
        jobs[n++] = plane_job(c, PL_W1, params + c.po.o[0], d.D, c.po.per_arm);
        jobs[n++] = plane_job(c, PL_W11, params + c.po.o[26], d.H, c.po.per_arm, params + c.po.o[27], c.po.per_arm);
    }
    if (p.chain_planes)
        for (int s = 0; s < PL_SMALL_LAYERS; ++s) {
            jobs[n++] = small_plane_job(c, params, s, false);
            jobs[n++] = small_plane_job(c, params, s, true);
        }
    return launch_presplit(c.stream, d.A, jobs, n, xbits ? &xb : nullptr);
}

int launch_dec_planes(const Ctx& c, const float* params) {
    const Plan& p = c.plan;
    const mmvae_dims& d = c.d;
    SplitJob jobs[6];
    int n = 0;
    if (p.fc11 == FC11_OUT_X3 || p.fc11 == FC11_OUT_BF16)
        jobs[n++] = plane_job(c, PL_W11, params + c.po.o[26], d.H, c.po.per_arm, params + c.po.o[27], c.po.per_arm);
    if (p.chain_planes)
        for (int s = PL_SMALL_DEC0; s < PL_SMALL_LAYERS; ++s) jobs[n++] = small_plane_job(c, params, s, false);
    return n ? launch_presplit(c.stream, d.A, jobs, n) : 0;
}

int launch_fc11_out_bf16(const Ctx& c, float* x_rec) {
    const mmvae_dims& d = c.d;
    Operand w{}, dp{};
    use_planes(c, w, PL_W11); use_planes(c, dp, PL_D10);
    Fc11OutArgs a{};
    a.wpl = w.pl; a.w_plane = w.pl_plane; a.w_arm = w.pl_arm;
    a.dpl = dp.pl; a.d_plane = dp.pl_plane; a.d_arm = dp.pl_arm;
    a.out = x_rec;
    a.B = d.B; a.D = d.D;
    const bool x3 = c.plan.fc11 == FC11_OUT_X3;
    const int blocks = cdiv(d.B, 128) * d.A, slots = (x3 ? 1 : 2) * 256, cap = min(64, cdiv(d.D, 32));
    int ks = 1;
    double best = 0.0;
    for (int k = 1; k <= cap; ++k) {
        const int nwg = blocks * k;
        const double eff = (double)nwg / (double)(cdiv(nwg, slots) * slots);
        if (nwg >= slots && eff >= 0.9) { ks = k; break; }
        if (eff > best + 1e-9) { best = eff; ks = k; }
    }
    a.KS = ks;
    const dim3 grid(cdiv(d.B, 128), ks, d.A);
    if (x3) hipLaunchKernelGGL((k_fc11_out<3, 7>), grid, dim3(256), 0, c.stream, a);
    else hipLaunchKernelGGL((k_fc11_out<1, 8>), grid, dim3(256), 0, c.stream, a);
    HIP_LAUNCH_CHECK("k_fc11_out");
    return 0;
}

static Operand x_operand(const Ctx& c, const float* x, int64_t xs, bool minor, int64_t* arm, int64_t* bits_arm) {
    const mmvae_dims& d = c.d;
    Operand o = minor ? kminor(x, d.D, d.D, d.B) : kmajor(x, d.D, d.B, d.D);
    if (c.dropout()) { o.bits = reinterpret_cast<const uint32_t*>(c.ws + c.lay.xbits); o.wpr = cdiv(d.D, 32); }
    if (c.plan.rowmap) { o.rowmap = reinterpret_cast<const unsigned*>(c.ws + c.lay.rowmap); o.nrec = c.x_nrows * c.x_ld; o.map_n = d.B; }
    if (c.plan.rowmap && c.plan.big != GEMM_X3 && c.x16) { o.ptr = reinterpret_cast<const float*>(c.x16); o.src16 = 1; }
    *arm = xs; *bits_arm = (int64_t)d.B * o.wpr;
    return o;
}

typedef void (*GemmKernel)(const GemmArgs);
struct SlabVariant { bool x3, aminor, bminor; int share, idx, s16; GemmKernel kernel; };
#define BF16_GEMM(AMINOR, BMINOR, IDX, S16) SlabVariant{false, AMINOR, BMINOR, 0, IDX, S16, k_bf16_gemm<AMINOR, BMINOR, IDX, S16>}
#define X3_GEMM(AMINOR, BMINOR, SHARE, IDX) SlabVariant{true, AMINOR, BMINOR, SHARE, IDX, 0, k_x3_gemm<AMINOR, BMINOR, SHARE, IDX>}
static const SlabVariant slab_variants[] = {
    BF16_GEMM(false, false, 0, 0), BF16_GEMM(false, false, 1, 0), BF16_GEMM(false, false, 1, 1), BF16_GEMM(false, false, 1, 3),
    X3_GEMM(false, false, 2, 0), X3_GEMM(false, false, 2, 1),
    BF16_GEMM(false, true, 0, 0),
    BF16_GEMM(true, true, 0, 0), BF16_GEMM(true, true, 2, 0), BF16_GEMM(true, true, 2, 2), BF16_GEMM(true, true, 2, 3),
    X3_GEMM(true, true, 1, 0), X3_GEMM(true, true, 1, 2),
    BF16_GEMM(true, true, 0, 1), X3_GEMM(true, true, 2, 0),
};
#undef BF16_GEMM
#undef X3_GEMM
static int launch_slab_gemm(const Ctx& c, const GemmArgs& g, int share, dim3 grid, const char* what) {
    const bool x3 = c.plan.big == GEMM_X3, aminor = g.a.kminor != 0, bminor = g.b.kminor != 0;
    const int idx = (g.a.rowmap ? 1 : 0) | (g.b.rowmap ? 2 : 0), s16 = (g.a.src16 ? 1 : 0) | (g.b.src16 ? 2 : 0);
    if (!x3) share = 0;
    for (const SlabVariant& v : slab_variants)
        if (v.x3 == x3 && v.aminor == aminor && v.bminor == bminor && v.share == share && v.idx == idx && v.s16 == s16) {
            hipLaunchKernelGGL(v.kernel, grid, dim3(x3 ? 512 : 256), 0, c.stream, g);
            HIP_LAUNCH_CHECK(what);
            return 0;
        }
    set_error("%s: no %s kernel for A k-%s, B k-%s, share %d, row map %d, bf16 source %d", what, x3 ? "k_x3_gemm" : "k_bf16_gemm",
              aminor ? "minor" : "major", bminor ? "minor" : "major", share, idx, s16);
    return MMVAE_E_LAUNCH;
}
static dim3 slab_grid(const Ctx& c, const GemmArgs& g, int paired) {
    return dim3(c.plan.big == GEMM_X3 ? cdiv(cdiv(paired, BT), 2) : cdiv(g.M, BT) * cdiv(g.N, BT), g.KS, g.A);
}

int launch_fc1_fwd_bf16(const Ctx& c, const float* params, const float* x, int64_t xs) {
    const mmvae_dims& d = c.d;
    GemmArgs g{};
    g.a = x_operand(c, x, xs, false, &g.a_arm, &g.a_bits_arm);
    g.b = kmajor(params + c.po.o[0], d.D, d.H, d.D); g.b_arm = c.po.per_arm;
    if (c.plan.big == GEMM_X3) use_planes(c, g.b, PL_W1);
    else if (g.a.src16 && c.plan.narrow) g.b_arm = read_slice0_bf16(c, g.b, PL_W1);
    g.M = d.B; g.N = d.H; g.K = d.D; g.KS = c.lay.sp.ks_fc1; g.A = d.A;
    g.so = SlabOut{c.ws + c.lay.fc1_slab, (int64_t)d.A * d.B * NP, (int64_t)d.B * NP, NP, d.B, d.H};
    return launch_slab_gemm(c, g, 2, slab_grid(c, g, d.B), "k_bf16_gemm<fc1>");
}

static GemmArgs fc11_args(const Ctx& c, const float* params, const float* x, int64_t xs, float* x_rec) {
    const mmvae_dims& d = c.d;
    const Layout& L = c.lay;
    GemmArgs g{};
    g.a = kmajor(c.ws + L.Dk[4], d.H, d.B, d.H);
    g.b = kmajor(params + c.po.o[26], d.H, d.D, d.H);
    g.M = d.B; g.N = d.D; g.K = d.H; g.KS = L.sp.ks_gd10; g.A = d.A; g.n11 = L.n11;
    g.fo = Fc11Out{params + c.po.o[27], x, c.ws + L.DZ11, x_rec, c.ws + L.fc11_part, c.fc11_coef(), d.B, d.D, nullptr, 0};
    if (c.plan.rowmap) {
        g.fo.xmap = reinterpret_cast<const unsigned*>(c.ws + L.rowmap);
        g.fo.x_nrec = c.x_nrows * c.x_ld;
    }
    g.fo_arm = (int64_t)d.B * d.D;
    g.fo_x_arm = xs;
    return g;
}
static SlabOut gd10_slab(const Ctx& c) {
    const mmvae_dims& d = c.d;
    return SlabOut{c.ws + c.lay.GD10_slab, (int64_t)d.A * d.B * d.H, (int64_t)d.B * d.H, d.H, d.B, d.H};
}

int launch_fc11_x3(const Ctx& c, const float* params, const float* x, int64_t xs) {
    const mmvae_dims& d = c.d;
    GemmArgs g = fc11_args(c, params, x, xs, nullptr);
    use_planes(c, g.b, PL_W11);
    use_planes(c, g.a, PL_D10);
    g.so = gd10_slab(c);
    launch_k(c, c.plan.fc11_fork_rides ? c.ev(EV_FORK) : nullptr, k_x3_fc11g, dim3(cdiv(d.B, 128), g.KS, d.A), dim3(256), 0, g);
    HIP_LAUNCH_CHECK("k_x3_fc11g");
    return 0;
}

int launch_fc11_bf16(const Ctx& c, const float* params, const float* x, int64_t xs, float* x_rec, int need_grad) {
    const mmvae_dims& d = c.d;
    if (int rc = zero_fc11_part(c)) return rc;
    if (!fc11_slots_fit(c.lay, d.B)) { set_error("fc11 bf16: loss partial slots"); return MMVAE_E_LAUNCH; }
    GemmArgs g = fc11_args(c, params, x, xs, x_rec);
    g.a_arm = (int64_t)d.B * d.H;
    g.b_arm = c.po.per_arm;
    g.bias_arm = c.po.per_arm;
    const dim3 grid(cdiv(d.B, BT), g.KS, d.A);
    if (!(need_grad && !x_rec)) {
        hipLaunchKernelGGL(k_bf16_fc11, grid, dim3(256), 0, c.stream, g);
        HIP_LAUNCH_CHECK("k_bf16_fc11");
        return 0;
    }
    g.so = gd10_slab(c);
    const hipEvent_t fork = c.plan.fc11_fork_rides ? c.ev(EV_FORK) : nullptr;
    const bool s16 = c.plan.dz11_bf16;
    if (s16) {
        g.fo.x = reinterpret_cast<const float*>(c.x16);
        g.fo_arm = (int64_t)d.B * d.D / 2;
        if (c.plan.narrow) g.b_arm = read_slice0_bf16(c, g.b, PL_W11, true);
    }
    static const GemmKernel variants[2][2] = {{k_bf16_fc11g<false, false>, nullptr},
                                              {k_bf16_fc11g<true, false>, k_bf16_fc11g<true, true>}};
    const GemmKernel kernel = variants[s16][g.b.src16 != 0];
    if (!kernel) { set_error("k_bf16_fc11g: no kernel for a bf16 W11 beside an fp32 x"); return MMVAE_E_LAUNCH; }
    launch_k(c, fork, kernel, grid, dim3(256), 0, g);
    HIP_LAUNCH_CHECK("k_bf16_fc11g");
    return 0;
}

int launch_gd10_bf16(const Ctx& c, const float* params) {
    const mmvae_dims& d = c.d;
    GemmArgs g{};
    g.a = kmajor(c.ws + c.lay.DZ11, d.D, d.B, d.D);
    g.a_arm = (int64_t)d.B * d.D;
    g.b = kminor(params + c.po.o[26], d.H, d.H, d.D);
    g.b_arm = c.po.per_arm;
    g.M = d.B; g.N = d.H; g.K = d.D; g.KS = c.lay.sp.ks_gd10; g.A = d.A;
    g.so = gd10_slab(c);
    return launch_slab_gemm(c, g, 0, slab_grid(c, g, 0), "k_bf16_gemm<gd10>");
}

int launch_dw1_bf16(const Ctx& c, const float* x, int64_t xs) {
    const mmvae_dims& d = c.d;
    const Layout& L = c.lay;
    GemmArgs g{};
    g.a = kminor(c.ws + L.DZ[1], d.H, d.H, d.B); g.a_arm = (int64_t)d.B * d.H;
    g.b = x_operand(c, x, xs, true, &g.b_arm, &g.b_bits_arm);
    if (c.plan.big == GEMM_X3) use_planes(c, g.a, PL_DZ1);
    else if (g.b.src16 && c.plan.narrow && c.plan.dz1_in_apply) g.a_arm = read_slice0_bf16(c, g.a, PL_DZ1);
    g.M = d.H; g.N = d.D; g.K = d.B; g.KS = L.sp.ks_dw; g.A = d.A;
    g.so = SlabOut{c.ws + L.dw1_slab, (int64_t)d.A * d.H * d.D, (int64_t)d.H * d.D, d.D, d.H, d.D};
    return launch_slab_gemm(c, g, 1, slab_grid(c, g, d.D), "k_bf16_gemm<dW1>");
}

int launch_dw11_bf16(const Ctx& c) {
    const mmvae_dims& d = c.d;
    const Layout& L = c.lay;
    GemmArgs g{};
    g.a = kminor(c.ws + L.DZ11, d.D, d.D, d.B); g.a_arm = (int64_t)d.B * d.D;
    g.b = kminor(c.ws + L.Dk[4], d.H, d.H, d.B); g.b_arm = (int64_t)d.B * d.H;
    g.b.ones_row = d.H;
    if (c.plan.big == GEMM_X3) use_planes(c, g.b, PL_D10);
    else if (c.plan.dz11_bf16) { g.a.src16 = 1; g.a_arm /= 2; }
    g.M = d.D; g.N = d.H + 1; g.K = d.B; g.KS = L.sp.ks_dw11; g.A = d.A;
    g.so = SlabOut{c.ws + L.dw11_slab, (int64_t)d.A * d.D * DW11_LD, (int64_t)d.D * DW11_LD, DW11_LD, d.D, d.H + 1};
    return launch_slab_gemm(c, g, 2, slab_grid(c, g, d.D), "k_bf16_gemm<dW11>");
}

int launch_dw_small_x3(const Ctx& c, const TnDescs& ts, int nsel) {
    const int KS = c.lay.sp.ks_small;
    hipLaunchKernelGGL(k_x3_small, dim3(cdiv(nsel * c.d.A, 2), KS), dim3(512), 0, c.stream, ts, nsel, c.d.A, c.d.B, KS);
    HIP_LAUNCH_CHECK("k_x3_small");
    return 0;
}

}
```

Measured before the change: 7.714 million cells/s.

## Precompute per-thread tile addressing, use buffer OOB for bounds, add maskless GEMM variants

Moves per-thread row/column and bit-mask offsets for tile loads into a PieceCtx computed once per kernel. Out-of-range pieces now read from an out-of-bounds buffer offset instead of clamping. Adds template variants that skip keep-mask loads when no dropout mask is present, and simplifies the ones-row and batch-norm handling. The epilogue becomes buffer stores with OOB masking, and the x3 kernel's interleaved two-group loop is restructured with explicit barriers. The aim is to cut address arithmetic, branch and register cost in the load and store paths, at the cost of more kernel variants and stricter launch checks.

```diff
diff --git a/distributed-vae_amd/csrc/gemm_bf16.hip b/distributed-vae_amd/csrc/gemm_bf16.hip
--- a/distributed-vae_amd/csrc/gemm_bf16.hip
+++ b/distributed-vae_amd/csrc/gemm_bf16.hip
@@ -52,12 +52,14 @@
     uint32_t wd[BITS ? NQ : 1];
 };
 
+constexpr unsigned PIECE_OOB = 0xFFFFFFF0u;
 struct OperandDev {
     __amdgpu_buffer_rsrc_t rs, rb;
     __amdgpu_buffer_rsrc_t rm;
     const unsigned* mp;
     int ld, rows, K, wpr, ones_row;
     bool bits;
+    unsigned nomask;
     float4 bn_sub, bn_mul;
 };
 template <bool KMINOR>
@@ -69,9 +71,10 @@
                                              (int)((o.rowmap ? o.map_n : 1) * 4), 0x00020000);
     d.mp = o.rowmap;
     d.bits = o.bits != nullptr;
+    d.nomask = d.bits ? 0u : 0xFFFFFFFFu;
     const int64_t nb = (KMINOR ? (int64_t)o.K : (int64_t)o.rows) * o.wpr;
     d.rb = __builtin_amdgcn_make_buffer_rsrc(const_cast<uint32_t*>(d.bits ? o.bits : reinterpret_cast<const uint32_t*>(o.ptr)), 0,
-                                             (int)((d.bits ? nb : 1) * 4), 0x00020000);
+                                             (int)((d.bits ? nb : 0) * 4), 0x00020000);
     d.ld = (int)o.ld; d.rows = o.rows; d.K = o.K; d.wpr = o.wpr; d.ones_row = o.ones_row;
     return d;
 }
@@ -81,54 +84,16 @@
     if (!KMINOR && NP != 1) { p = q; h = 0; }
     else { p = q >> 1; h = q & 1; }
 }
-template <bool KMINOR, bool BITS = true, int NP = 1>
-__device__ __forceinline__ void quad_load(TileRegsT<BITS, Eng<NP>::NQ>& t, const OperandDev& o, int r0, int k0, int kend, int q) {
-    const int tid = threadIdx.x & 255;
-    int p, h;
-    piece_ph<KMINOR, NP>(q, p, h);
-    int off, woff;
-    if (!KMINOR) {
-        const int row = r0 + (tid >> 3) + 32 * p;
-        const int rc = min(row, o.rows - 1);
-        const int k = k0 + ((tid & 7) + 8 * h) * 4;
-        const bool ok = row < o.rows && k + 3 < kend && k + 3 < o.K;
-        off = rc * o.ld + (ok ? k : 0);
-        woff = rc * o.wpr + ((ok ? k : 0) >> 5);
-    } else {
-        const int k = k0 + 2 * ((tid >> 5) + 8 * p) + h;
-        const int kc = min(k, o.K - 1);
-        const int row = r0 + (tid & 31) * 4;
-        off = kc * o.ld + (row < o.ld ? row : 0);
-        woff = kc * o.wpr + (min(row, o.rows - 1) >> 5);
-    }
-    t.v[q] = __builtin_bit_cast(float4, __builtin_amdgcn_raw_buffer_load_b128(o.rs, off * 4, 0, 0));
-    if constexpr (BITS) t.wd[q] = o.bits ? (uint32_t)__builtin_amdgcn_raw_buffer_load_b32(o.rb, woff * 4, 0, 0) : 0xFFFFFFFFu;
-}
-
-template <bool KMINOR, int NP>
-__device__ __forceinline__ void quad_load_idx(TileRegsT<true, Eng<NP>::NQ>& t, const OperandDev& o, int r0, int k0, int kend, int q,
-                                              const unsigned (&ro)[Eng<NP>::NQ]) {
-    const int tid = threadIdx.x & 255;
-    int p, h;
-    piece_ph<KMINOR, NP>(q, p, h);
-    int off, woff;
-    if (!KMINOR) {
-        const int row = r0 + (tid >> 3) + 32 * p;
-        const int rc = min(row, o.rows - 1);
-        const int k = k0 + ((tid & 7) + 8 * h) * 4;
-        const bool ok = row < o.rows && k + 3 < kend && k + 3 < o.K;
-        off = (int)ro[q] + (ok ? k : 0);
-        woff = rc * o.wpr + ((ok ? k : 0) >> 5);
-    } else {
-        const int k = k0 + 2 * ((tid >> 5) + 8 * p) + h;
-        const int kc = min(k, o.K - 1);
-        const int row = r0 + (tid & 31) * 4;
-        off = (int)ro[q] + (row < o.ld ? row : 0);
-        woff = kc * o.wpr + (min(row, o.rows - 1) >> 5);
-    }
-    t.v[q] = __builtin_bit_cast(float4, __builtin_amdgcn_raw_buffer_load_b128(o.rs, off * 4, 0, 0));
-    t.wd[q] = o.bits ? (uint32_t)__builtin_amdgcn_raw_buffer_load_b32(o.rb, woff * 4, 0, 0) : 0xFFFFFFFFu;
-}
+struct PieceCtx {
+    unsigned vb;
+    unsigned vr[4];
+    unsigned wb;
+    int lim;
+    int sh;
+    int kl;
+    int one;
+    int li;
+};
 typedef unsigned mapw4 __attribute__((ext_vector_type(4)));
 typedef const mapw4 __attribute__((address_space(4)))* map4_ptr;
 template <int NP>
@@ -149,23 +114,65 @@
         ro[q] = hi ? mr.s[p][2 + h] : mr.s[p][h];
     }
 }
-template <int NP>
-__device__ __forceinline__ void ro_init(unsigned (&ro)[Eng<NP>::NQ], const OperandDev& o, int r0) {
+template <bool KMINOR, int NP, bool IDX = false>
+__device__ __forceinline__ PieceCtx piece_ctx(const OperandDev& o, int r0) {
     const int tid = threadIdx.x & 255;
-#pragma unroll
-    for (int q = 0; q < Eng<NP>::NQ; ++q) {
-        int p, h;
-        piece_ph<false, NP>(q, p, h);
-        ro[q] = (unsigned)__builtin_amdgcn_raw_buffer_load_b32(o.rm, min(r0 + (tid >> 3) + 32 * p, o.rows - 1) * 4, 0, 0);
-    }
+    PieceCtx c = {};
+    if (!KMINOR) {
+        const int kq = tid & 7, rr = tid >> 3, row = r0 + rr;
+        c.vb = ((unsigned)row * (unsigned)o.ld + kq * 4u) * 4u;
+        if constexpr (IDX) {
+#pragma unroll
+            for (int p = 0; p < 4; ++p)
+                c.vr[p] = ((unsigned)__builtin_amdgcn_raw_buffer_load_b32(o.rm, min(row + 32 * p, o.rows - 1) * 4, 0, 0) + kq * 4u) * 4u;
+        }
+        c.wb = (unsigned)row * (unsigned)o.wpr * 4u;
+        c.lim = o.rows - row;
+        c.sh = kq * 4;
+        c.kl = kq * 4 + 3;
+        c.li = rr * Eng<NP>::LDB + kq * 2;
+    } else {
+        const int r4 = (tid & 31) * 4, kp = tid >> 5, row = r0 + r4;
+        c.vb = IDX ? row * 4u : (2u * kp * (unsigned)o.ld + row) * 4u;
+        c.wb = (2u * kp * (unsigned)o.wpr + (row >> 5)) * 4u;
+        c.lim = (1 << min(max(o.rows - row, 0), 4)) - 1;
+        c.sh = row & 31;
+        c.kl = 2 * kp;
+        const int e = o.ones_row - row;
+        c.one = (o.ones_row >= 0 && e >= 0 && e < 4) ? 1 << e : 0;
+        c.li = (2 * kp * Eng<NP>::LDK + r4) >> 1;
+    }
+    return c;
+}
+template <bool KMINOR, bool BITS = true, int NP = 1, bool IDX = false>
+__device__ __forceinline__ void quad_load(TileRegsT<BITS, Eng<NP>::NQ>& t, const OperandDev& o, const PieceCtx& c, int k0, int kend, int q,
+                                          const unsigned* ro = nullptr) {
+    int p, h;
+    piece_ph<KMINOR, NP>(q, p, h);
+    bool ok;
+    unsigned vo, so, swo;
+    if (!KMINOR) {
+        ok = 32 * p < c.lim && k0 + 32 * h + c.kl < kend;
+        vo = IDX ? c.vr[p] : c.vb;
+        so = IDX ? (unsigned)(k0 + 32 * h) * 4u : (32u * p * (unsigned)o.ld + k0 + 32 * h) * 4u;
+        swo = (32u * p * (unsigned)o.wpr + (k0 >> 5) + h) * 4u;
+    } else {
+        const int ks = k0 + 16 * p + h;
+        ok = c.lim != 0 && ks + c.kl < kend;
+        vo = IDX ? ro[q] * 4u + c.vb : c.vb;
+        so = IDX ? 0u : (unsigned)ks * (unsigned)o.ld * 4u;
+        swo = (unsigned)ks * (unsigned)o.wpr * 4u;
+    }
+    t.v[q] = __builtin_bit_cast(float4, __builtin_amdgcn_raw_buffer_load_b128(o.rs, (int)(ok ? vo + so : PIECE_OOB), 0, 0));
+    if constexpr (BITS) t.wd[q] = (uint32_t)__builtin_amdgcn_raw_buffer_load_b32(o.rb, (int)(ok ? c.wb + swo : PIECE_OOB), 0, 0);
 }
 template <bool KMINOR, int NP>
-__device__ __forceinline__ void idx_begin(unsigned (&ro)[Eng<NP>::NQ], MapRegs<NP>& mr, const OperandDev& o, int r0, int kfirst) {
+__device__ __forceinline__ void idx_begin(unsigned (&ro)[Eng<NP>::NQ], MapRegs<NP>& mr, const OperandDev& o, int kfirst) {
     if constexpr (KMINOR) {
         map_request<NP>(mr, o, kfirst);
         map_offsets<NP>(ro, mr);
         map_request<NP>(mr, o, kfirst + Eng<NP>::KT);
-    } else ro_init<NP>(ro, o, r0);
+    }
 }
 template <bool KMINOR, int NP>
 __device__ __forceinline__ void idx_next(unsigned (&ro)[Eng<NP>::NQ], MapRegs<NP>& mr, const OperandDev& o, int kld) {
@@ -174,47 +181,44 @@
         map_request<NP>(mr, o, kld + Eng<NP>::KT);
     }
 }
-template <bool KMINOR, bool BITS = true, int NP = 1, bool BN = false>
-__device__ __forceinline__ void quad_store(unsigned* __restrict__ T, const TileRegsT<BITS, Eng<NP>::NQ>& t, const OperandDev& o, int r0,
+template <bool KMINOR, bool BITS = true, int NP = 1, bool BN = false, bool ONES = BN>
+__device__ __forceinline__ void quad_store(unsigned* __restrict__ T, const TileRegsT<BITS, Eng<NP>::NQ>& t, const OperandDev& o, const PieceCtx& c,
                                            int k0, int kend, int q) {
-    constexpr int LDBv = Eng<NP>::LDB, PLANE = Eng<NP>::PLANE;
-    const int tid = threadIdx.x & 255;
+    constexpr int PLANE = Eng<NP>::PLANE;
     int p, h;
     piece_ph<KMINOR, NP>(q, p, h);
-    float x[4];
+    const float4 v = t.v[q];
+    float x[4] = {v.x, v.y, v.z, v.w};
     int idx;
     if (!KMINOR) {
-        const int kq = tid & 7, rr = tid >> 3;
-        const int row = r0 + rr + 32 * p;
-        const int k = k0 + (kq + 8 * h) * 4;
-        const bool ok = row < o.rows && k + 3 < kend && k + 3 < o.K;
-        const int nib = ok ? (BITS ? (int)(t.wd[q] >> (k & 31)) : 0xF) : 0;
-        const float4 v = t.v[q];
-        const float vv[4] = {v.x, v.y, v.z, v.w};
-#pragma unroll
-        for (int e = 0; e < 4; ++e) x[e] = __uint_as_float(__float_as_uint(vv[e]) & (unsigned)__builtin_amdgcn_sbfe(nib, e, 1));
-        idx = (rr + 32 * p) * LDBv + (kq + 8 * h) * 2;
+        if constexpr (BITS) {
+            const int nib = (int)((t.wd[q] | o.nomask) >> c.sh);
+#pragma unroll
+            for (int e = 0; e < 4; ++e) x[e] = __uint_as_float(__float_as_uint(x[e]) & (unsigned)__builtin_amdgcn_sbfe(nib, e, 1));
+        }
+        idx = c.li + 32 * p * Eng<NP>::LDB + 16 * h;
     } else {
-        const int r4 = (tid & 31) * 4, kp = tid >> 5;
-        const int kl = 2 * (kp + 8 * p) + h, k = k0 + kl;
-        const bool kok = k < kend && k < o.K;
-        const int nrow = min(max(o.rows - (r0 + r4), 0), 4);
-        const int nib = kok ? ((BITS ? (int)(t.wd[q] >> ((r0 + r4) & 31)) : 0xF) & ((1 << nrow) - 1)) : 0;
-        const float4 v = t.v[q];
-        const float vv[4] = {v.x, v.y, v.z, v.w};
-#pragma unroll
-        for (int e = 0; e < 4; ++e) x[e] = __uint_as_float(__float_as_uint(vv[e]) & (unsigned)__builtin_amdgcn_sbfe(nib, e, 1));
-        if constexpr (BN) {
-            const float sb[4] = {o.bn_sub.x, o.bn_sub.y, o.bn_sub.z, o.bn_sub.w}, ml[4] = {o.bn_mul.x, o.bn_mul.y, o.bn_mul.z, o.bn_mul.w};
-#pragma unroll
-            for (int e = 0; e < 4; ++e) x[e] = ((nib >> e) & 1) ? (x[e] - sb[e]) * ml[e] : 0.f;
-        }
-        if (o.ones_row >= 0) {
-#pragma unroll
-            for (int e = 0; e < 4; ++e)
-                if (kok && r0 + r4 + e == o.ones_row) x[e] = 1.f;
-        }
-        idx = (kl * Eng<NP>::LDK + r4) >> 1;
+        const int kt = 16 * p + h;
+        int nib = BITS ? (int)((t.wd[q] | o.nomask) >> c.sh) & c.lim : c.lim;
+        int one = c.one;
+        if constexpr (ONES) {
+            const bool kok = k0 + kt + c.kl < kend;
+            nib = kok ? nib : 0;
+            one = kok ? one : 0;
+        }
+#pragma unroll
+        for (int e = 0; e < 4; ++e) {
+            const unsigned m = (unsigned)__builtin_amdgcn_sbfe(nib, e, 1);
+            if constexpr (BN) {
+                const float sb[4] = {o.bn_sub.x, o.bn_sub.y, o.bn_sub.z, o.bn_sub.w}, ml[4] = {o.bn_mul.x, o.bn_mul.y, o.bn_mul.z, o.bn_mul.w};
+                x[e] = __uint_as_float(__float_as_uint((x[e] - sb[e]) * ml[e]) & m);
+            } else x[e] = __uint_as_float(__float_as_uint(x[e]) & m);
+            if constexpr (ONES) {
+                const unsigned m1 = (unsigned)__builtin_amdgcn_sbfe(one, e, 1);
+                x[e] = __uint_as_float((__float_as_uint(x[e]) & ~m1) | (__float_as_uint(1.f) & m1));
+            }
+        }
+        idx = c.li + ((kt * Eng<NP>::LDK) >> 1);
     }
     if constexpr (NP == 1) {
         uint2 w;
@@ -294,14 +298,16 @@
 
 template <bool KMINOR, bool BITS = true, int NP = 1>
 __device__ __forceinline__ void tile_load(TileRegsT<BITS, Eng<NP>::NQ>& t, const OperandDev& o, int r0, int k0, int kend) {
-#pragma unroll
-    for (int q = 0; q < Eng<NP>::NQ; ++q) quad_load<KMINOR, BITS, NP>(t, o, r0, k0, kend, q);
+    const PieceCtx c = piece_ctx<KMINOR, NP>(o, r0);
+#pragma unroll
+    for (int q = 0; q < Eng<NP>::NQ; ++q) quad_load<KMINOR, BITS, NP>(t, o, c, k0, kend, q);
 }
 template <bool KMINOR, bool BITS = true, int NP = 1>
 __device__ __forceinline__ void tile_store(unsigned* __restrict__ T, const TileRegsT<BITS, Eng<NP>::NQ>& t, const OperandDev& o, int r0,
                                            int k0, int kend) {
-#pragma unroll
-    for (int q = 0; q < Eng<NP>::NQ; ++q) quad_store<KMINOR, BITS, NP>(T, t, o, r0, k0, kend, q);
+    const PieceCtx c = piece_ctx<KMINOR, NP>(o, r0);
+#pragma unroll
+    for (int q = 0; q < Eng<NP>::NQ; ++q) quad_store<KMINOR, BITS, NP>(T, t, o, c, k0, kend, q);
 }
 
 typedef short s16x4 __attribute__((ext_vector_type(4)));
@@ -334,11 +340,11 @@
 }
 template <bool KMINOR>
 __device__ __forceinline__ void plane_load(PlaneRegs& t, const PlaneDev& o, int r0, int k0, int j) {
-    const int tid = threadIdx.x & 255, pl = j >> 1, id = tid + 256 * (j & 1);
-    int off;
-    if (!KMINOR) off = pl * o.plane + (r0 + (id >> 2)) * o.ld + k0 + 8 * (id & 3);
-    else off = pl * o.plane + (k0 + (id >> 4)) * o.ld + r0 + 8 * (id & 15);
-    t.v[j] = __builtin_bit_cast(u32x4v, __builtin_amdgcn_raw_buffer_load_b128(o.rs, off * 2, 0, 0));
+    const int tid = threadIdx.x & 255, pl = j >> 1, hi = j & 1;
+    int vo, so;
+    if (!KMINOR) { vo = (tid >> 2) * o.ld + 8 * (tid & 3); so = pl * o.plane + (r0 + 64 * hi) * o.ld + k0; }
+    else { vo = (tid >> 4) * o.ld + 8 * (tid & 15); so = pl * o.plane + (k0 + 16 * hi) * o.ld + r0; }
+    t.v[j] = __builtin_bit_cast(u32x4v, __builtin_amdgcn_raw_buffer_load_b128(o.rs, vo * 2, so * 2, 0));
 }
 template <bool KMINOR>
 __device__ __forceinline__ void plane_store(unsigned* __restrict__ T, const PlaneRegs& t, int j) {
@@ -481,23 +487,30 @@
     }
 }
 
+constexpr unsigned TILE_OOB = 0x80000000u;
+__device__ __forceinline__ void tile_out(float* out, int ld, int M, int N, const f32x16 (&acc)[2][2], int m0, int n0, int wm, int wn, int lane) {
+    const int rows = __builtin_amdgcn_readfirstlane(min(max(M - m0, 0), BT));
+    const __amdgpu_buffer_rsrc_t rs = __builtin_amdgcn_make_buffer_rsrc(out + (int64_t)m0 * ld, 0, rows * ld * 4, 0x00020000);
+    const unsigned ldb = (unsigned)ld * 4u;
+    const unsigned row_l = (unsigned)(64 * wm + 4 * (lane >> 5)) * ldb;
+#pragma unroll
+    for (int j = 0; j < 2; ++j) {
+        const int col = n0 + 64 * wn + 32 * j + (lane & 31);
+        const unsigned o_lane = col < N ? row_l + (unsigned)col * 4u : TILE_OOB;
+#pragma unroll
+        for (int i = 0; i < 2; ++i)
+#pragma unroll
+            for (int r = 0; r < 16; ++r) {
+                const float v = acc[i][j][r];
+                __builtin_amdgcn_raw_buffer_store_b32(__float_as_uint(v), rs, (int)(o_lane + (unsigned)(32 * i + acc_row(r, 0)) * ldb), 0, 0);
+            }
+    }
+}
 __device__ __forceinline__ void gemm_epilogue(const GemmArgs& g, const f32x16 (&acc)[2][2], int m0, int n0, int wm, int wn, int lane, int arm) {
-    const int l31 = lane & 31;
-    float* out = g.so.out + (int64_t)blockIdx.y * g.so.ks_stride + (int64_t)arm * g.so.arm_stride;
-#pragma unroll
-    for (int i = 0; i < 2; ++i)
-#pragma unroll
-        for (int j = 0; j < 2; ++j) {
-            const int col = n0 + 64 * wn + 32 * j + l31;
-#pragma unroll
-            for (int r = 0; r < 16; ++r) {
-                const int row = m0 + 64 * wm + 32 * i + acc_row(r, lane);
-                if (row < g.so.M && col < g.so.N) out[(int64_t)row * g.so.ld + col] = acc[i][j][r];
-            }
-        }
-}
-
-template <bool AMINOR, bool BMINOR, int IDX = 0, int S16 = 0>
+    tile_out(g.so.out + (int64_t)blockIdx.y * g.so.ks_stride + (int64_t)arm * g.so.arm_stride, g.so.ld, g.so.M, g.so.N, acc, m0, n0, wm, wn, lane);
+}
+
+template <bool AMINOR, bool BMINOR, int IDX = 0, int S16 = 0, bool XMASK = true>
 __global__ __launch_bounds__(256, 2) void k_bf16_gemm(const GemmArgs g_in) {
     const GemmArgs g = g_in;
     __shared__ __attribute__((aligned(16))) unsigned As[2][BT * LDB];
@@ -516,12 +529,17 @@
     const int kb = (int)(((int64_t)blockIdx.y * nkt) / g.KS) * KT;
     const int ke = min(g.K, (int)(((int64_t)(blockIdx.y + 1) * nkt) / g.KS) * KT);
     f32x16 acc[2][2] = {{zero16(), zero16()}, {zero16(), zero16()}};
-    TileRegsT<true> ta, tb;
+    constexpr bool ABITS = XMASK && !AMINOR && !BMINOR, BBITS = XMASK && AMINOR && BMINOR;
+    TileRegsT<ABITS> ta;
+    TileRegsT<BBITS> tb;
     OctRegs t16a, t16b;
     unsigned ro[Eng<1>::NQ] = {};
     MapRegs<1> mr = {};
     static_assert(IDX == 0 || S16 == 0 || (S16 & IDX) != 0, "row map and bf16 storage: the indexed operand (x) is a bf16 one");
     constexpr bool A16 = (S16 & 1) != 0, B16 = (S16 & 2) != 0;
+    constexpr bool AIDX = IDX == 1 && !A16, BIDX = IDX == 2 && !B16;
+    constexpr bool BONES = AMINOR && BMINOR && IDX == 0;
+    const PieceCtx ca = piece_ctx<AMINOR, 1, AIDX>(oa, m0), cb = piece_ctx<BMINOR, 1, BIDX>(ob, n0);
     auto stage = [&](unsigned* Ad, unsigned* Bd, int kst, int kld, auto load_tag) __attribute__((always_inline)) {
         constexpr bool LOAD = decltype(load_tag)::value;
         if constexpr (LOAD && IDX == 1 && AMINOR) {
@@ -540,11 +558,8 @@
                     if constexpr (LOAD) oct_load<AMINOR, IDX == 1>(t16a, oa, m0, kld, ke, q, ro);
                 }
             } else {
-                quad_store<AMINOR>(Ad, ta, oa, m0, kst, ke, q);
-                if constexpr (LOAD) {
-                    if constexpr (IDX == 1) quad_load_idx<AMINOR, 1>(ta, oa, m0, kld, ke, q, ro);
-                    else quad_load<AMINOR>(ta, oa, m0, kld, ke, q);
-                }
+                quad_store<AMINOR, ABITS>(Ad, ta, oa, ca, kst, ke, q);
+                if constexpr (LOAD) quad_load<AMINOR, ABITS, 1, AIDX>(ta, oa, ca, kld, ke, q, ro);
             }
             if constexpr (B16) {
                 if (q < 4) {
@@ -552,11 +567,8 @@
                     if constexpr (LOAD) oct_load<BMINOR, IDX == 2>(t16b, ob, n0, kld, ke, q, ro);
                 }
             } else {
-                quad_store<BMINOR>(Bd, tb, ob, n0, kst, ke, q);
-                if constexpr (LOAD) {
-                    if constexpr (IDX == 2) quad_load_idx<BMINOR, 1>(tb, ob, n0, kld, ke, q, ro);
-                    else quad_load<BMINOR>(tb, ob, n0, kld, ke, q);
-                }
+                quad_store<BMINOR, BBITS, 1, false, BONES>(Bd, tb, ob, cb, kst, ke, q);
+                if constexpr (LOAD) quad_load<BMINOR, BBITS, 1, BIDX>(tb, ob, cb, kld, ke, q, ro);
             }
         }
     };
@@ -574,11 +586,14 @@
             }
 #pragma unroll
             for (int q = 0; q < 4; ++q) oct_load<MINOR, IDXD>(t16, o, r0, kb, ke, q, ro);
-        } else if constexpr (IDXD) {
-            idx_begin<MINOR, 1>(ro, mr, o, r0, kb);
-#pragma unroll
-            for (int q = 0; q < Eng<1>::NQ; ++q) quad_load_idx<MINOR, 1>(ISA ? ta : tb, o, r0, kb, ke, q, ro);
-        } else tile_load<MINOR>(ISA ? ta : tb, o, r0, kb, ke);
+        } else {
+            if constexpr (IDXD) idx_begin<MINOR, 1>(ro, mr, o, kb);
+#pragma unroll
+            for (int q = 0; q < Eng<1>::NQ; ++q) {
+                if constexpr (ISA) quad_load<MINOR, ABITS, 1, IDXD>(ta, o, ca, kb, ke, q, ro);
+                else quad_load<MINOR, BBITS, 1, IDXD>(tb, o, cb, kb, ke, q, ro);
+            }
+        }
     };
     if (kb < ke) {
         first(VecTag{});
@@ -604,21 +619,22 @@
 #define X3_DEPTH 1
 #endif
 static_assert(X3_DEPTH == 1 || X3_DEPTH == 2, "one or two K tiles in flight");
-template <bool AMINOR, bool BMINOR, int SHARE, int IDX = 0>
+template <bool AMINOR, bool BMINOR, int SHARE, int IDX = 0, bool MASK = true>
 __global__ __launch_bounds__(512, 1) void k_x3_gemm(const GemmArgs g_in) {
     static_assert(SHARE == 1 || SHARE == 2, "the two tiles of a block share one operand");
+    static_assert(IDX == 0 || IDX == (SHARE == 2 ? 1 : 2), "the row map belongs to the operand that is read as fp32");
     typedef Eng<3> E;
     constexpr int KTv = E::KT;
+    constexpr bool FMINOR = SHARE == 2 ? AMINOR : BMINOR, PMINOR = SHARE == 2 ? BMINOR : AMINOR, IDXD = IDX != 0;
     const GemmArgs g = g_in;
     __shared__ __attribute__((aligned(16))) unsigned As[2][3 * E::PLANE];
     __shared__ __attribute__((aligned(16))) unsigned Bs[2][3 * E::PLANE];
-    const int arm = blockIdx.z, grp = threadIdx.x >> 8, tid = threadIdx.x & 255, lane = tid & 63, wv = tid >> 6, wm = wv >> 1, wn = wv & 1;
-    Operand oa_h = g.a, ob_h = g.b;
-    oa_h.ptr += (int64_t)arm * g.a_arm;
-    ob_h.ptr += (int64_t)arm * g.b_arm;
-    if (oa_h.bits) oa_h.bits += (int64_t)arm * g.a_bits_arm;
-    if (ob_h.bits) ob_h.bits += (int64_t)arm * g.b_bits_arm;
-    const OperandDev oa = make_operand_dev<AMINOR>(oa_h), ob = make_operand_dev<BMINOR>(ob_h);
+    const int grp = __builtin_amdgcn_readfirstlane((int)threadIdx.x >> 8);
+    const int arm = blockIdx.z, tid = threadIdx.x & 255, lane = tid & 63, wv = tid >> 6, wm = wv >> 1, wn = wv & 1;
+    Operand of_h = SHARE == 2 ? g.a : g.b;
+    of_h.ptr += (int64_t)arm * (SHARE == 2 ? g.a_arm : g.b_arm);
+    if (of_h.bits) of_h.bits += (int64_t)arm * (SHARE == 2 ? g.a_bits_arm : g.b_bits_arm);
+    const OperandDev of = make_operand_dev<FMINOR>(of_h);
     const int tiles_m = cdiv(g.M, BT), tiles_n = cdiv(g.N, BT);
     const int bi = blockIdx.x;
     int tm, tn;
@@ -626,88 +642,53 @@
     else { tm = bi % tiles_m; tn = 2 * (bi / tiles_m) + grp; }
     const bool active = tm < tiles_m && tn < tiles_n;
     const int m0 = tm * BT, n0 = tn * BT;
+    const int rf = SHARE == 2 ? m0 : n0, rp = SHARE == 2 ? n0 : m0;
     const int nkt = cdiv(g.K, KTv);
     const int kb = (int)(((int64_t)blockIdx.y * nkt) / g.KS) * KTv;
     const int ke = min(g.K, (int)(((int64_t)(blockIdx.y + 1) * nkt) / g.KS) * KTv);
     const int n = ke > kb ? cdiv(ke - kb, KTv) : 0;
     f32x16 acc[2][2] = {{zero16(), zero16()}, {zero16(), zero16()}};
     constexpr int DEPTH = X3_DEPTH;
-    TileRegsT<true, E::NQ> ta_[DEPTH], tb_[DEPTH];
+    TileRegsT<MASK, E::NQ> tf_[DEPTH];
     unsigned ro[E::NQ] = {};
     MapRegs<3> mr = {};
     PlaneRegs ps;
-    constexpr bool APL = SHARE == 1, BPL = SHARE == 2;
     const PlaneDev dp = make_plane_dev(SHARE == 1 ? g.a : g.b, arm);
-    const bool do_a = SHARE != 1 || grp == 0, do_b = SHARE != 2 || grp == 0;
-    auto stage = [&](unsigned* Ad, unsigned* Bd, int kst, int kld, int kpl, auto load_tag, auto loadp_tag, auto slot_tag) __attribute__((always_inline)) {
+    const PieceCtx cf = piece_ctx<FMINOR, 3, IDXD>(of, rf);
+    auto stage = [&](unsigned* Fd, unsigned* Pd, int kst, int kld, int kpl, auto load_tag, auto loadp_tag, auto slot_tag) __attribute__((always_inline)) {
         constexpr bool LOAD = decltype(load_tag)::value, LOADP = decltype(loadp_tag)::value;
         constexpr int SLOT = decltype(slot_tag)::value;
-        TileRegsT<true, E::NQ>& ta = ta_[SLOT];
-        TileRegsT<true, E::NQ>& tb = tb_[SLOT];
-        if constexpr (LOAD && IDX == 1) idx_next<AMINOR, 3>(ro, mr, oa, kld);
-        if constexpr (LOAD && IDX == 2) idx_next<BMINOR, 3>(ro, mr, ob, kld);
+        TileRegsT<MASK, E::NQ>& tf = tf_[SLOT];
+        if constexpr (LOAD && IDXD) idx_next<FMINOR, 3>(ro, mr, of, kld);
+        auto planes = [&](int i) __attribute__((always_inline)) {
+            if (grp == 0) {
+                plane_store<PMINOR>(Pd, ps, i);
+                if constexpr (LOADP) plane_load<PMINOR>(ps, dp, rp, kpl, i);
+            }
+        };
 #pragma unroll
         for (int i = 0; i < 6; ++i) {
-            if constexpr (APL) {
-                if (do_a) {
-                    plane_store<AMINOR>(Ad, ps, i);
-                    if constexpr (LOADP) plane_load<AMINOR>(ps, dp, m0, kpl, i);
-                }
-            } else if (i < E::NQ) {
-                if (do_a) {
-                    quad_store<AMINOR, true, 3>(Ad, ta, oa, m0, kst, ke, i);
-                    if constexpr (LOAD) {
-                        if constexpr (IDX == 1) quad_load_idx<AMINOR, 3>(ta, oa, m0, kld, ke, i, ro);
-                        else quad_load<AMINOR, true, 3>(ta, oa, m0, kld, ke, i);
-                    }
-                }
-            }
-            if constexpr (BPL) {
-                if (do_b) {
-                    plane_store<BMINOR>(Bd, ps, i);
-                    if constexpr (LOADP) plane_load<BMINOR>(ps, dp, n0, kpl, i);
-                }
-            } else if (i < E::NQ) {
-                if (do_b) {
-                    quad_store<BMINOR, true, 3>(Bd, tb, ob, n0, kst, ke, i);
-                    if constexpr (LOAD) {
-                        if constexpr (IDX == 2) quad_load_idx<BMINOR, 3>(tb, ob, n0, kld, ke, i, ro);
-                        else quad_load<BMINOR, true, 3>(tb, ob, n0, kld, ke, i);
-                    }
-                }
-            }
+            if constexpr (SHARE == 1) planes(i);
+            if (i < E::NQ) {
+                quad_store<FMINOR, MASK, 3>(Fd, tf, of, cf, kst, ke, i);
+                if constexpr (LOAD) quad_load<FMINOR, MASK, 3, IDXD>(tf, of, cf, kld, ke, i, ro);
+            }
+            if constexpr (SHARE == 2) planes(i);
         }
     };
     auto first = [&](auto slot_tag, int k) __attribute__((always_inline)) {
         constexpr int SLOT = decltype(slot_tag)::value;
-        TileRegsT<true, E::NQ>& ta = ta_[SLOT];
-        TileRegsT<true, E::NQ>& tb = tb_[SLOT];
-        if constexpr (APL) {
-            if (SLOT == 0 && do_a) {
-#pragma unroll
-                for (int i = 0; i < 6; ++i) plane_load<AMINOR>(ps, dp, m0, k, i);
-            }
-        } else if (do_a) {
-            if constexpr (IDX == 1) {
-                if constexpr (SLOT == 0) idx_begin<AMINOR, 3>(ro, mr, oa, m0, k);
-                else idx_next<AMINOR, 3>(ro, mr, oa, k);
-#pragma unroll
-                for (int q = 0; q < E::NQ; ++q) quad_load_idx<AMINOR, 3>(ta, oa, m0, k, ke, q, ro);
-            } else tile_load<AMINOR, true, 3>(ta, oa, m0, k, ke);
-        }
-        if constexpr (BPL) {
-            if (SLOT == 0 && do_b) {
-#pragma unroll
-                for (int i = 0; i < 6; ++i) plane_load<BMINOR>(ps, dp, n0, k, i);
-            }
-        } else if (do_b) {
-            if constexpr (IDX == 2) {
-                if constexpr (SLOT == 0) idx_begin<BMINOR, 3>(ro, mr, ob, n0, k);
-                else idx_next<BMINOR, 3>(ro, mr, ob, k);
-#pragma unroll
-                for (int q = 0; q < E::NQ; ++q) quad_load_idx<BMINOR, 3>(tb, ob, n0, k, ke, q, ro);
-            } else tile_load<BMINOR, true, 3>(tb, ob, n0, k, ke);
-        }
+        TileRegsT<MASK, E::NQ>& tf = tf_[SLOT];
+        if (SLOT == 0 && grp == 0) {
+#pragma unroll
+            for (int i = 0; i < 6; ++i) plane_load<PMINOR>(ps, dp, rp, k, i);
+        }
+        if constexpr (IDXD) {
+            if constexpr (SLOT == 0) idx_begin<FMINOR, 3>(ro, mr, of, k);
+            else idx_next<FMINOR, 3>(ro, mr, of, k);
+        }
+#pragma unroll
+        for (int q = 0; q < E::NQ; ++q) quad_load<FMINOR, MASK, 3, IDXD>(tf, of, cf, k, ke, q, ro);
     };
     if (active && n > 0) {
         first(std::integral_constant<int, 0>{}, kb);
@@ -715,29 +696,33 @@
             if (n > 1) first(std::integral_constant<int, DEPTH - 1>{}, kb + KTv);
         }
     }
-    for (int p = 0; p <= 2 * n; ++p) {
-        const int q = p - grp;
-        if (active && q >= 0 && q < 2 * n) {
-            const int t = q >> 1, k0 = kb + t * KTv;
-            unsigned* const Ad = As[SHARE == 1 ? (t & 1) : grp];
-            unsigned* const Bd = Bs[SHARE == 2 ? (t & 1) : grp];
-            if (q & 1) {
-                mfma_ktile<AMINOR, BMINOR, 3>(acc, Ad, Bd, wm, wn, lane);
-            } else {
-                const bool more = t + DEPTH < n, morep = t + 1 < n;
-                const int kld = k0 + DEPTH * KTv, kpl = k0 + KTv;
-                auto go = [&](auto slot_tag) __attribute__((always_inline)) {
-                    if (more) stage(Ad, Bd, k0, kld, kpl, VecTag{}, VecTag{}, slot_tag);
-                    else if (morep) stage(Ad, Bd, k0, k0, kpl, ScalarTag{}, VecTag{}, slot_tag);
-                    else stage(Ad, Bd, k0, k0, k0, ScalarTag{}, ScalarTag{}, slot_tag);
-                };
-                if (DEPTH == 1 || !(t & 1)) go(std::integral_constant<int, 0>{});
-                else go(std::integral_constant<int, DEPTH - 1>{});
-            }
-        }
+    if (!active) {
+        for (int p = 0; p <= 2 * n; ++p) __syncthreads();
+        return;
+    }
+    if (grp == 1) __syncthreads();
+    for (int t = 0; t < n; ++t) {
+        const int k0 = kb + t * KTv;
+        unsigned* const Ad = As[SHARE == 1 ? (t & 1) : grp];
+        unsigned* const Bd = Bs[SHARE == 2 ? (t & 1) : grp];
+        unsigned* const Fd = SHARE == 2 ? Ad : Bd;
+        unsigned* const Pd = SHARE == 2 ? Bd : Ad;
+        const bool more = t + DEPTH < n, morep = t + 1 < n;
+        const int kld = k0 + DEPTH * KTv, kpl = k0 + KTv;
+        auto go = [&](auto slot_tag) __attribute__((always_inline)) {
+            if (more) stage(Fd, Pd, k0, kld, kpl, VecTag{}, VecTag{}, slot_tag);
+            else if (morep) stage(Fd, Pd, k0, k0, kpl, ScalarTag{}, VecTag{}, slot_tag);
+            else stage(Fd, Pd, k0, k0, k0, ScalarTag{}, ScalarTag{}, slot_tag);
+        };
+        if (DEPTH == 1 || !(t & 1)) go(std::integral_constant<int, 0>{});
+        else go(std::integral_constant<int, DEPTH - 1>{});
         __syncthreads();
-    }
-    if (active) gemm_epilogue(g, acc, m0, n0, wm, wn, lane, arm);
+        mfma_ktile<AMINOR, BMINOR, 3>(acc, Ad, Bd, wm, wn, lane);
+        __builtin_amdgcn_sched_barrier(0);
+        __syncthreads();
+    }
+    if (grp == 0) __syncthreads();
+    gemm_epilogue(g, acc, m0, n0, wm, wn, lane, arm);
 }
 
 __global__ __launch_bounds__(256, 2) void k_bf16_fc11(const GemmArgs g_in) {
@@ -1374,7 +1359,8 @@
     constexpr int KTv = E::KT;
     __shared__ __attribute__((aligned(16))) unsigned As[2][3 * E::PLANE];
     __shared__ __attribute__((aligned(16))) unsigned Bs[2][3 * E::PLANE];
-    const int grp = threadIdx.x >> 8, tid = threadIdx.x & 255, lane = tid & 63, wv = tid >> 6, wm = wv >> 1, wn = wv & 1;
+    const int grp = __builtin_amdgcn_readfirstlane((int)threadIdx.x >> 8);
+    const int tid = threadIdx.x & 255, lane = tid & 63, wv = tid >> 6, wm = wv >> 1, wn = wv & 1;
     const int unit = 2 * blockIdx.x + grp;
     const bool active = unit < ndesc * A;
     const int di = active ? unit % ndesc : 0, arm = active ? unit / ndesc : 0;
@@ -1402,46 +1388,42 @@
     const int n = ke > kb ? cdiv(ke - kb, KTv) : 0;
     f32x16 acc[2][2] = {{zero16(), zero16()}, {zero16(), zero16()}};
     TileRegsT<false, E::NQ> ta, tb;
+    const PieceCtx ca = piece_ctx<true, 3>(oa, 0), cb = piece_ctx<true, 3>(ob, 0);
     unsigned* const Ad = As[grp];
     unsigned* const Bd = Bs[grp];
     auto stage = [&](int kst, int kld, auto load_tag) __attribute__((always_inline)) {
         constexpr bool LOAD = decltype(load_tag)::value;
 #pragma unroll
         for (int i = 0; i < E::NQ; ++i) {
-            quad_store<true, false, 3>(Ad, ta, oa, 0, kst, ke, i);
-            if constexpr (LOAD) quad_load<true, false, 3>(ta, oa, 0, kld, ke, i);
-            quad_store<true, false, 3, true>(Bd, tb, ob, 0, kst, ke, i);
-            if constexpr (LOAD) quad_load<true, false, 3>(tb, ob, 0, kld, ke, i);
+            quad_store<true, false, 3>(Ad, ta, oa, ca, kst, ke, i);
+            if constexpr (LOAD) quad_load<true, false, 3>(ta, oa, ca, kld, ke, i);
+            quad_store<true, false, 3, true>(Bd, tb, ob, cb, kst, ke, i);
+            if constexpr (LOAD) quad_load<true, false, 3>(tb, ob, cb, kld, ke, i);
         }
     };
     if (active && n > 0) {
-        tile_load<true, false, 3>(ta, oa, 0, kb, ke);
-        tile_load<true, false, 3>(tb, ob, 0, kb, ke);
-    }
-    for (int p = 0; p <= 2 * n; ++p) {
-        const int q = p - grp;
-        if (active && q >= 0 && q < 2 * n) {
-            const int k0 = kb + (q >> 1) * KTv;
-            if (q & 1) mfma_ktile<true, true, 3>(acc, Ad, Bd, wm, wn, lane);
-            else if (k0 + KTv < ke) stage(k0, k0 + KTv, VecTag{});
-            else stage(k0, k0, ScalarTag{});
-        }
+#pragma unroll
+        for (int i = 0; i < E::NQ; ++i) {
+            quad_load<true, false, 3>(ta, oa, ca, kb, ke, i);
+            quad_load<true, false, 3>(tb, ob, cb, kb, ke, i);
+        }
+    }
+    if (!active) {
+        for (int p = 0; p <= 2 * n; ++p) __syncthreads();
+        return;
+    }
+    if (grp == 1) __syncthreads();
+    for (int t = 0; t < n; ++t) {
+        const int k0 = kb + t * KTv;
+        if (k0 + KTv < ke) stage(k0, k0 + KTv, VecTag{});
+        else stage(k0, k0, ScalarTag{});
         __syncthreads();
-    }
-    if (!active) return;
-    float* out = d.out + (int64_t)blockIdx.y * d.out_ks_stride + (int64_t)arm * d.out_arm_stride;
-    const int ncols = d.Nv + d.q_ones, l31 = lane & 31;
-#pragma unroll
-    for (int i = 0; i < 2; ++i)
-#pragma unroll
-        for (int j = 0; j < 2; ++j) {
-            const int col = 64 * wn + 32 * j + l31;
-#pragma unroll
-            for (int r = 0; r < 16; ++r) {
-                const int row = 64 * wm + 32 * i + acc_row(r, lane);
-                if (row < d.Mv && col < ncols) out[(int64_t)row * d.ldo + col] = acc[i][j][r];
-            }
-        }
+        mfma_ktile<true, true, 3>(acc, Ad, Bd, wm, wn, lane);
+        __builtin_amdgcn_sched_barrier(0);
+        __syncthreads();
+    }
+    if (grp == 0) __syncthreads();
+    tile_out(d.out + (int64_t)blockIdx.y * d.out_ks_stride + (int64_t)arm * d.out_arm_stride, d.ldo, d.Mv, d.Nv + d.q_ones, acc, 0, 0, wm, wn, lane);
 }
 
 static Operand kmajor(const float* p, int64_t ld, int rows, int K) {
@@ -1582,16 +1564,16 @@
 }
 
 typedef void (*GemmKernel)(const GemmArgs);
-struct SlabVariant { bool x3, aminor, bminor; int share, idx, s16; GemmKernel kernel; };
-#define BF16_GEMM(AMINOR, BMINOR, IDX, S16) SlabVariant{false, AMINOR, BMINOR, 0, IDX, S16, k_bf16_gemm<AMINOR, BMINOR, IDX, S16>}
-#define X3_GEMM(AMINOR, BMINOR, SHARE, IDX) SlabVariant{true, AMINOR, BMINOR, SHARE, IDX, 0, k_x3_gemm<AMINOR, BMINOR, SHARE, IDX>}
+struct SlabVariant { bool x3, aminor, bminor; int share, idx, s16, mask; GemmKernel kernel; };
+#define BF16_GEMM(AMINOR, BMINOR, IDX, S16, MASK) SlabVariant{false, AMINOR, BMINOR, 0, IDX, S16, MASK, k_bf16_gemm<AMINOR, BMINOR, IDX, S16, MASK != 0>}
+#define X3_GEMM(AMINOR, BMINOR, SHARE, IDX, MASK) SlabVariant{true, AMINOR, BMINOR, SHARE, IDX, 0, MASK, k_x3_gemm<AMINOR, BMINOR, SHARE, IDX, MASK != 0>}
 static const SlabVariant slab_variants[] = {
-    BF16_GEMM(false, false, 0, 0), BF16_GEMM(false, false, 1, 0), BF16_GEMM(false, false, 1, 1), BF16_GEMM(false, false, 1, 3),
-    X3_GEMM(false, false, 2, 0), X3_GEMM(false, false, 2, 1),
-    BF16_GEMM(false, true, 0, 0),
-    BF16_GEMM(true, true, 0, 0), BF16_GEMM(true, true, 2, 0), BF16_GEMM(true, true, 2, 2), BF16_GEMM(true, true, 2, 3),
-    X3_GEMM(true, true, 1, 0), X3_GEMM(true, true, 1, 2),
-    BF16_GEMM(true, true, 0, 1), X3_GEMM(true, true, 2, 0),
+    BF16_GEMM(false, false, 0, 0, 1), BF16_GEMM(false, false, 1, 0, 1), BF16_GEMM(false, false, 1, 1, 1), BF16_GEMM(false, false, 1, 3, 1),
+    X3_GEMM(false, false, 2, 0, 1), X3_GEMM(false, false, 2, 1, 1), X3_GEMM(false, false, 2, 0, 0),
+    BF16_GEMM(false, true, 0, 0, 0),
+    BF16_GEMM(true, true, 0, 0, 1), BF16_GEMM(true, true, 2, 0, 1), BF16_GEMM(true, true, 2, 2, 1), BF16_GEMM(true, true, 2, 3, 1),
+    X3_GEMM(true, true, 1, 0, 1), X3_GEMM(true, true, 1, 2, 1), X3_GEMM(true, true, 1, 0, 0),
+    BF16_GEMM(true, true, 0, 0, 0), BF16_GEMM(true, true, 0, 1, 0), X3_GEMM(true, true, 2, 0, 0),
 };
 #undef BF16_GEMM
 #undef X3_GEMM
@@ -1599,14 +1581,30 @@
     const bool x3 = c.plan.big == GEMM_X3, aminor = g.a.kminor != 0, bminor = g.b.kminor != 0;
     const int idx = (g.a.rowmap ? 1 : 0) | (g.b.rowmap ? 2 : 0), s16 = (g.a.src16 ? 1 : 0) | (g.b.src16 ? 2 : 0);
     if (!x3) share = 0;
-    for (const SlabVariant& v : slab_variants)
-        if (v.x3 == x3 && v.aminor == aminor && v.bminor == bminor && v.share == share && v.idx == idx && v.s16 == s16) {
-            hipLaunchKernelGGL(v.kernel, grid, dim3(x3 ? 512 : 256), 0, c.stream, g);
-            HIP_LAUNCH_CHECK(what);
-            return 0;
-        }
-    set_error("%s: no %s kernel for A k-%s, B k-%s, share %d, row map %d, bf16 source %d", what, x3 ? "k_x3_gemm" : "k_bf16_gemm",
-              aminor ? "minor" : "major", bminor ? "minor" : "major", share, idx, s16);
+    const Operand& f = share == 1 ? g.b : g.a;
+    if (x3 && (!(share == 1 ? g.a : g.b).pl || (share == 1 ? g.a : g.b).bits || f.ones_row >= 0)) {
+        set_error("%s: k_x3_gemm takes the shared operand as slice planes and masks / extends neither it nor the other by a ones row", what);
+        return MMVAE_E_LAUNCH;
+    }
+    if (!x3 && (g.a.ones_row >= 0 || (g.b.ones_row >= 0 && !(aminor && bminor && idx == 0)))) {
+        set_error("%s: k_bf16_gemm extends only the B operand of a k-minor x k-minor product without a row map by a ones row", what);
+        return MMVAE_E_LAUNCH;
+    }
+    if (!x3 && ((g.a.bits && (aminor || bminor)) || (g.b.bits && !(aminor && bminor)))) {
+        set_error("%s: k_bf16_gemm takes a keep-mask on A of a k-major x k-major or on B of a k-minor x k-minor product only", what);
+        return MMVAE_E_LAUNCH;
+    }
+    const int mask = (x3 ? f.bits != nullptr : g.a.bits || g.b.bits) ? 1 : 0;
+    for (int pass = 0; pass < (x3 ? 1 : 2); ++pass)
+        for (const SlabVariant& v : slab_variants)
+            if (v.x3 == x3 && v.aminor == aminor && v.bminor == bminor && v.share == share && v.idx == idx && v.s16 == s16 &&
+                (pass == 0 ? v.mask == mask : v.mask >= mask)) {
+                hipLaunchKernelGGL(v.kernel, grid, dim3(x3 ? 512 : 256), 0, c.stream, g);
+                HIP_LAUNCH_CHECK(what);
+                return 0;
+            }
+    set_error("%s: no %s kernel for A k-%s, B k-%s, share %d, row map %d, bf16 source %d, mask %d", what, x3 ? "k_x3_gemm" : "k_bf16_gemm",
+              aminor ? "minor" : "major", bminor ? "minor" : "major", share, idx, s16, mask);
     return MMVAE_E_LAUNCH;
 }
 static dim3 slab_grid(const Ctx& c, const GemmArgs& g, int paired) {
```

New measurement: 8.128 million cells/s (median of 6 runs). +5.4%, better.
